# zyc-123/InstanceDiff

Hardware: AMD Instinct MI355X
Metric: denoising steps/sec (256x256 bs16) (higher is better)
Workload: dtype f32; 1 GPU; 256x256 1-ch synthetic, 1000-step reverse chain, batch 16 per GPU, 2 UNet fwd + reverse update per step; global_batch=16, parallelism=replicas x1 (no collective)

## Files before the change

### include/idiff.h

```cpp
#ifndef IDIFF_H
#define IDIFF_H

#include <stdint.h>

#ifdef __cplusplus
extern "C" {
#endif

#define IDIFF_OK 0
#define IDIFF_E_BADARG (-1)
#define IDIFF_E_UNSUPPORTED (-2)
#define IDIFF_E_HIP (-3)

typedef void* idiff_stream_t;

const char* idiff_last_error(void);
int idiff_version(void);
int64_t idiff_launch_count(void);
int idiff_device_info(int* num_cu, int* wave_size, char* arch_name, int arch_name_len);

#define IDIFF_CONV_NORMAL 0
#define IDIFF_CONV_UPSAMPLE2 1
#define IDIFF_CONV_UNSHUFFLE2 2

typedef struct {
    const float* src0;
    const float* src1;
    int64_t src0_bstride, src1_bstride;
    int32_t C0, C1;
    int32_t B, Hin, Win;
    int32_t mode;
    int32_t ks;
    int32_t Cout;
    const float* wpk;
    const float* bias;
    const float* pro_a;
    const float* pro_b;
    float* out;
    int64_t out_bstride;
    const float* res;
    int64_t res_bstride;
    const float* vec;
    const float* aux;
    int64_t aux_bstride;
    const float* aux_a;
    const float* aux_b;
    float* stats;
    const float* wwino;
    const float* wwino4;
    const float* gn_gamma;
    const float* gn_beta;
    const float* gn_film;
    int64_t gn_film_ld;
    float gn_eps;
    int32_t gn_groups;
    float* gn_out_a;
    float* gn_out_b;
    float* gn_mean_rstd;
    int32_t algo_request;
    const void* wx3;
    const void* wbf16;
    int32_t operands;
} idiff_conv_desc;

int idiff_conv2d_num_tiles(int Hout, int Wout);
int idiff_conv2d_fwd(const idiff_conv_desc* d, idiff_stream_t stream);
#define IDIFF_CONV_ALGO_DIRECT 0
#define IDIFF_CONV_ALGO_WINOGRAD 1
#define IDIFF_CONV_ALGO_STREAM1X1 2
#define IDIFF_CONV_ALGO_WINOGRAD4 3
#define IDIFF_CONV_ALGO_WINOGRAD4H 4
#define IDIFF_CONV_ALGO_X3 5
#define IDIFF_CONV_ALGO_BF16 6
int idiff_conv2d_last_algo(void);
int idiff_conv2d_plan(const idiff_conv_desc* d);
long long idiff_conv1x1_x3_image_bytes(int Cout, int Cin);
int idiff_pack_conv1x1_x3(const float* w, void* image, int Cout, int Cin, idiff_stream_t stream);
int idiff_pack_conv_weight(const float* w, float* wpk, int Cout, int Cin, int ks, idiff_stream_t stream);
int idiff_pack_conv_weight_T(const float* w, float* wpk, int Cout, int Cin, int ks, idiff_stream_t stream);
int idiff_pack_conv_weight_wino(const float* w, float* wwino, int Cout, int Cin, int transpose, idiff_stream_t stream);
int idiff_pack_conv_weight_wino4(const float* w, float* wwino4, int Cout, int Cin, int transpose, idiff_stream_t stream);
long long idiff_conv_weight_bf16_bytes(int Cout, int Cin, int transpose);
int idiff_pack_conv_weight_bf16(const float* w, void* image, int Cout, int Cin, int transpose, idiff_stream_t stream);

int idiff_gn_finalize(const float* stats, int ntiles, int B, int C, int groups, int HW, const float* gamma,
                      const float* beta, const float* film, int64_t film_ld, float eps, float* out_a, float* out_b,
                      float* mean_rstd, idiff_stream_t stream);

int idiff_affine_silu_add(const float* h, int64_t h_bstride, const float* a, const float* b, const float* res,
                          int64_t res_bstride, const float* vec, float* out, int64_t out_bstride, int B, int C, int HW,
                          idiff_stream_t stream);

#define IDIFF_ACT_NONE 0
#define IDIFF_ACT_SILU 1
#define IDIFF_ACT_GELU 2
int idiff_linear_fwd(const float* x, int64_t ldx, const float* w, int64_t ldw, const float* bias, const float* res,
                     int64_t ldr, const float* gscale, float* out, int64_t ldo, int R, int K, int N, int act_in,
                     int act_out, idiff_stream_t stream);
int idiff_linear_t_fwd(const float* x, int64_t ldx, const float* wT, int64_t ldw, const float* bias, const float* res,
                       int64_t ldr, const float* gscale, float* out, int64_t ldo, int R, int K, int N, int act_in,
                       int act_out, idiff_stream_t stream);
#define IDIFF_LINEAR_MAX_GROUPS 16
typedef struct {
    const float* x;
    int64_t ldx;
    const float* wT;
    int64_t ldw;
    const float* bias;
    const float* res;
    int64_t ldr;
    const float* gscale;
    float* out;
    int64_t ldo;
    const float* ln_g;
    const float* ln_b;
    float ln_eps;
    int32_t R, K, N, act_in, act_out;
} idiff_linear_group;
int idiff_linear_t_grouped_fwd(const idiff_linear_group* groups, int ngroups, idiff_stream_t stream);
int idiff_linear_t_ln_fwd(const float* x, int64_t ldx, const float* ln_g, const float* ln_b, float ln_eps, const float* wT,
                          int64_t ldw, const float* bias, const float* res, int64_t ldr, const float* gscale, float* out,
                          int64_t ldo, int R, int K, int N, int act_out, idiff_stream_t stream);
int idiff_linear_t_heads_fwd(const float* x, int64_t ldx, int64_t x_hs, const float* wT, int64_t ldw, int64_t w_hs,
                             const float* bias, int64_t b_hs, float* out, int64_t ldo, int64_t o_hs, int R, int K, int N,
                             int heads, idiff_stream_t stream);
int idiff_smm_memproj_fwd(const float* feat, int64_t feat_bstride, const float* ln1_g, const float* ln1_b,
                          const float* wpk, const float* bias, const float* ln2_g, const float* ln2_b, float* out, int B,
                          int C, int N, float eps, idiff_stream_t stream);
int idiff_smm_memproj_compact_fwd(const float* feat, int64_t feat_bstride, const float* ln1_g, const float* ln1_b,
                                  const float* gram, const float* hvec, float evar, float* out, int B, int C, int N, int Cm,
                                  float eps1, float eps2, idiff_stream_t stream);
int idiff_smm_memproj_compact_train_fwd(const float* feat, int64_t feat_bstride, const float* ln1_g, const float* ln1_b, const float* gram,
                                        const float* hvec, const float* evar_dev, float* out, int B, int C, int N, int Cm, float eps1,
                                        float eps2, idiff_stream_t stream);
int64_t idiff_smm_memproj_compact_bwd_ws_floats(int B, int C, int N);
int idiff_smm_memproj_compact_bwd(const float* feat, int64_t feat_bstride, const float* ln1_g, const float* ln1_b, const float* gram,
                                  const float* hvec, const float* evar_dev, const float* dm, float* dfeat, int64_t dfeat_bstride,
                                  float* dparams, float* ws, int B, int C, int N, int Cm, float eps1, float eps2, idiff_stream_t stream);
#define IDIFF_MEMPROJ_MAX_GROUPS 4
typedef struct idiff_memproj_group {
    const float* feat;
    int64_t feat_bstride;
    const float *ln1_g, *ln1_b, *gram, *hvec;
    float evar;
    float* out;
    int32_t C, N, Cm;
} idiff_memproj_group;
int idiff_smm_memproj_compact_grouped_fwd(const idiff_memproj_group* groups, int ngroups, int B, float eps1, float eps2,
                                          idiff_stream_t stream);
int idiff_layernorm_rows_fwd(const float* x, int64_t ldx, const float* gamma, const float* beta, float* out,
                             int64_t ldo, int R, int C, float eps, float* mean_rstd, idiff_stream_t stream);
int idiff_time_embed_fwd(const float* t, const float* freqs, int B, int dim, float* out, idiff_stream_t stream);
int idiff_time_mlp_fwd(const float* t, const float* freqs, const float* w0, const float* b0, const float* w2, const float* b2, float* out,
                       int B, int dim, int hid, int nout, idiff_stream_t stream);

int idiff_chan_layernorm_fwd(const float* x, int64_t x_bstride, const float* gamma, const float* beta, float* out,
                             int64_t out_bstride, int B, int C, int HW, float eps, float* mean_rstd,
                             idiff_stream_t stream);

int idiff_attn_self_fwd(const float* qkv, float* out, float* lse, int B, int C, int N, int heads, float scale,
                        idiff_stream_t stream);
int idiff_attn_self_bf16_fwd(const float* qkv, float* out, int B, int C, int N, int heads, float scale, idiff_stream_t stream);
int idiff_attn_self_f16_fwd(const float* qkv, float* out, int B, int C, int N, int heads, float scale, idiff_stream_t stream);
int idiff_attn_ctx_fwd(const float* q, const float* k, const float* v, float* out, int B, int C, int N, int M,
                       int heads, float scale, idiff_stream_t stream);
int idiff_attn_tokens_fwd(const float* q, const float* k, const float* v, float* out, int B, int Nq, int M, int C,
                          int heads, float scale, int64_t ldq, int64_t ldkv, idiff_stream_t stream);
int idiff_attn_tokens_bwd(const float* q, const float* k, const float* v, const float* d_o, float* dq, float* dk, float* dv, int B, int Nq,
                          int M, int C, int heads, float scale, int64_t ldq, int64_t ldkv, int64_t ldo, int64_t lddq, int64_t lddkv,
                          idiff_stream_t stream);
int idiff_attn_tokens_grouped_fwd(const float* const* q, const float* const* k, const float* const* v, float* const* out, int ngroups,
                                  int B, int Nq, int M, int C, int heads, float scale, int64_t ldq, int64_t ldkv, idiff_stream_t stream);
int idiff_attn_tokens_f16_fwd(const float* q, const float* k, const float* v, float* out, int B, int Nq, int M, int C, int heads, float scale,
                              int64_t ldq, int64_t ldkv, idiff_stream_t stream);
int64_t idiff_smm_xattn_kv_f16_ws_floats(int B, int N);
int idiff_smm_xattn_kv_f16_fwd(const float* q, const float* k, const float* v, float* out, float* ws, int B, int Nq, int heads, int C, int N,
                               float scale, idiff_stream_t stream);
int64_t idiff_smm_xattn_ws_floats(int B, int Nq, int heads, int Cm, int N);
int idiff_smm_xattn_fwd(const float* qf, const float* mem, float* o, float* ws, int B, int Nq, int heads, int Cm,
                        int N, float scale, idiff_stream_t stream);
#define IDIFF_XATTN_MAX_GROUPS 8
typedef struct idiff_xattn_group {
    const float* qf;
    const float* mem;
    float* o;
    float* ws;
    int32_t Cm, N;
} idiff_xattn_group;
int idiff_smm_xattn_grouped_fwd(const idiff_xattn_group* groups, int ngroups, int B, int Nq, int heads, float scale,
                                idiff_stream_t stream);
int idiff_smm_xattn_lse_fwd(const float* qf, const float* mem, float* o, float* lse, float* ws, int B, int rows, int N, float scale,
                            idiff_stream_t stream);
int idiff_smm_xattn_bwd(const float* qf, const float* mem, const float* o, const float* lse, const float* d_o, float* dqf, float* dmem,
                        int accumulate, float* ws, int B, int rows, int N, float scale, idiff_stream_t stream);
int idiff_smm_xattn_cm_lse_fwd(const float* qf, const float* mem, float* o, float* lse, float* ws, int B, int rows, int Cm, int N,
                               float scale, idiff_stream_t stream);
int idiff_smm_xattn_cm_bwd(const float* qf, const float* mem, const float* o, const float* lse, const float* d_o, float* dqf, float* dmem,
                           int accumulate, float* ws, int B, int rows, int Cm, int N, float scale, idiff_stream_t stream);
int idiff_scoremap_fwd(const float* feat, int64_t feat_bstride, const float* tv, float* out, const int32_t* idx,
                       float* sel, int B, int C, int HW, int K, idiff_stream_t stream);
#define IDIFF_SCOREMAP_MAX_GROUPS 4
typedef struct idiff_scoremap_group {
    const float* feat;
    int64_t feat_bstride;
    const float* tv;
    float* out;
    float* sel;
    int32_t C, HW;
} idiff_scoremap_group;
int idiff_scoremap_grouped_fwd(const idiff_scoremap_group* groups, int ngroups, const int32_t* idx, int B, int K, idiff_stream_t stream);
int idiff_conv3x3_select_fwd(const float* x, int64_t x_bstride, const float* w, const float* bias, const int32_t* idx, float* out,
                             int B, int C, int K, int H, int W, idiff_stream_t stream);
int64_t idiff_conv3x3_select_bwd_ws_floats(int B, int C, int H, int W);
int idiff_conv3x3_select_bwd(const float* x, int64_t x_bstride, const float* w, const int32_t* idx, const float* dpred, float* dx,
                             int64_t dx_bstride, float* dw, float* db, float* ws, int B, int C, int K, int H, int W, idiff_stream_t stream);
int idiff_gather_channel(const float* x, const int32_t* idx, float* out, int B, int C, int HW, idiff_stream_t stream);

#define IDIFF_SDE_STEP 0
#define IDIFF_SDE_MEAN 1
#define IDIFF_SDE_ODE 2
int idiff_irsde_reverse_step(const float* x, const float* mu, const float* noise_pred, const float* z, float* x_out,
                             int64_t n, float theta, float sigma, float sigma_bar, float dt, float sqrt_dt, int mode,
                             uint64_t seed, uint64_t offset, idiff_stream_t stream);
#define IDIFF_IRSDE_SCORE_FROM_NOISE 0
#define IDIFF_IRSDE_MU_BAR 1
#define IDIFF_IRSDE_DRIFT 2
#define IDIFF_IRSDE_REV_DRIFT 3
#define IDIFF_IRSDE_DISPERSION 4
#define IDIFF_IRSDE_STEP_MEAN 5
#define IDIFF_IRSDE_STEP_SDE 6
#define IDIFF_IRSDE_FORWARD_STEP 7
#define IDIFF_IRSDE_OPT_STEP 8
#define IDIFF_IRSDE_REAL_NOISE 9
#define IDIFF_IRSDE_REAL_SCORE 10
#define IDIFF_IRSDE_INIT_FROM_NOISE 11
#define IDIFF_IRSDE_RANDOM_STATES 12
#define IDIFF_IRSDE_NUM_OPS 13
int idiff_irsde_map(int op, const float* a, const float* b, const float* z, const float* mu, float mu_scalar, float* out, int B,
                    int64_t per_sample, const float* coef_dev, const float* k, uint64_t seed, uint64_t offset,
                    idiff_stream_t stream);
int idiff_drift_reverse_step(const float* x, const float* r_hat, const float* e_hat, const float* z, const float* cond,
                             float* x_out, float* xa_out, int64_t n, float a, float b, float c, uint64_t seed,
                             uint64_t offset, idiff_stream_t stream);
int idiff_drift_reverse_step_dev(float* x, const float* r_hat, const float* e_hat, const float* z_base, const float* cond,
                                 float* xa, int64_t n, const float* coef, int Tp1, const int32_t* state, uint64_t seed,
                                 uint64_t nper, uint64_t offset_base, idiff_stream_t stream);
int idiff_drift_reverse_step2_dev(float* x, const float* r_hat, const float* e_hat, float* r_prev, float* e_prev, const float* z_base,
                                  const float* cond, float* xa, int64_t n, const float* coef5, int Tp1, const int32_t* state,
                                  uint64_t seed, uint64_t nper, uint64_t offset_base, idiff_stream_t stream);
int idiff_randn_members(float* out, int R, int64_t n_s, const uint64_t* members_dev, uint64_t seed, uint64_t j, idiff_stream_t stream);
int idiff_ensemble_init(const float* cond, float* cond_rep, float* x, float* xa, int B, int S, int64_t n_s, const uint64_t* members_dev,
                        float sigma, uint64_t seed, idiff_stream_t stream);
int idiff_chain_begin(const float* cond_in, float* cond, float* x, float* xa, int B, int S, int64_t n_s, int64_t row0, int R,
                      const uint64_t* members_dev, float sigma, uint64_t seed, uint64_t offset, int32_t* state, float* tdev, int t0,
                      int calls0, idiff_stream_t stream);
int idiff_drift_reverse_step_members_dev(float* x, const float* r_hat, const float* e_hat, float* r_prev, float* e_prev, const float* z_base,
                                         const float* cond, float* xa, int R, int64_t n_s, const float* coef, int coef_rows, int Tp1,
                                         const int32_t* state, const uint64_t* members_dev, uint64_t seed, idiff_stream_t stream);
int idiff_ensemble_stats(const float* x, float* mean, float* std_out, int B, int S, int64_t n_s, idiff_stream_t stream);
int idiff_ensemble_order_stats(const float* x, float* out, int B, int S, int64_t n_s, const int32_t* ks_host, int nk, int algo,
                               idiff_stream_t stream);
int idiff_interval_coverage(const float* lo, const float* hi, const float* target, int32_t* counts, int32_t* ws, int B, int64_t n_s,
                            idiff_stream_t stream);
int64_t idiff_interval_coverage_ws_ints(int B, int64_t n_s);
int idiff_ensemble_scores(const float* x, const float* target, float* crps_map, double* sums, int32_t* counts, void* ws, int B, int S,
                          int64_t n_s, idiff_stream_t stream);
int64_t idiff_ensemble_scores_ws_bytes(int B, int S);
int idiff_tile_gather(const float* full, float* tiles, int B, int C, int H, int W, int ny, int nx, int Ph, int Pw, const int32_t* ytab,
                      const int32_t* xtab, idiff_stream_t stream);
int idiff_drift_reverse_step_tiled_dev(float* x, const float* r_tiles, const float* e_tiles, float* r_prev, float* e_prev, const float* z_base,
                                       const float* cond, float* x_tiles, float* xa_tiles, int B, int C, int H, int W, int ny, int nx, int Ph,
                                       int Pw, const int32_t* ytab, const float* ywt, const int32_t* xtab, const float* xwt, const float* coef,
                                       int coef_rows, int Tp1, const int32_t* state, uint64_t seed, uint64_t nper, uint64_t offset_base,
                                       idiff_stream_t stream);
int idiff_drift_reverse_step_tiled_members_dev(float* x, const float* r_tiles, const float* e_tiles, float* r_prev, float* e_prev,
                                               const float* z_base, const float* cond, float* x_tiles, float* xa_tiles, int R, int C, int H,
                                               int W, int ny, int nx, int Ph, int Pw, const int32_t* ytab, const float* ywt,
                                               const int32_t* xtab, const float* xwt, const float* coef, int coef_rows, int Tp1,
                                               const int32_t* state, const uint64_t* members_dev, uint64_t seed, idiff_stream_t stream);
int idiff_step_state_advance(int32_t* state, float* tdev, int B, int T, int t_stop, idiff_stream_t stream);
int idiff_step_state_advance_table(int32_t* state, float* tdev, int B, const int32_t* next_t, int Tp1, int t_first, int t_stop,
                                   idiff_stream_t stream);
int idiff_dropout(const float* x, float* out, int64_t n, float p, uint64_t seed, uint64_t offset, idiff_stream_t stream);
int idiff_randn(float* out, int64_t n, uint64_t seed, uint64_t offset, idiff_stream_t stream);
int idiff_philox_raw(uint32_t* out, int64_t ncounters, uint64_t seed, uint64_t offset, idiff_stream_t stream);
int idiff_axpby(const float* x, const float* y, float* out, int64_t n, float alpha, float beta, idiff_stream_t stream);
int idiff_sum_n(const float* const* srcs, const int64_t* src_bstrides, int nsrc, float* out, int64_t out_bstride, int B,
                int64_t per_sample, idiff_stream_t stream);
int idiff_gather_segments(const void* segs_dev, int nseg, int64_t nblocks, float* dst, idiff_stream_t stream);
int idiff_gather_segments_acc(const void* segs_dev, int nseg, int64_t nblocks, float* dst, idiff_stream_t stream);
int idiff_mix3_per_sample(const float* x0, const float* cond, const float* eps, const float* c0, const float* c1,
                          const float* c2, float* out, int B, int64_t per_sample, idiff_stream_t stream);


int64_t idiff_conv2d_wgrad_ws_floats(const idiff_conv_desc* d);
int idiff_conv2d_wgrad(const idiff_conv_desc* d, const float* dy, int64_t dy_bstride, float* dw, int accumulate, float* ws,
                       idiff_stream_t stream);
int idiff_conv2d_wgrad_last_algo(void);
int idiff_sumpool2x2(const float* x, float* out, int64_t planes, int h, int w, idiff_stream_t stream);
int idiff_pixel_shuffle2(const float* x, float* out, int B, int C, int h, int w, idiff_stream_t stream);
int idiff_plane_sum(const float* x, int64_t x_bstride, float* out_bc, int B, int C, int HW, idiff_stream_t stream);
int idiff_batch_sum(const float* in_bc, float* out_c, int B, int C, int accumulate, idiff_stream_t stream);

int64_t idiff_gn_silu_bwd_ws_floats(int B, int C, int groups);
int idiff_gn_silu_bwd(const float* dy, int64_t dy_bstride, const float* h, int64_t h_bstride, const float* a, const float* b,
                      const float* mean_rstd, const float* gamma, const float* beta, const float* film, int64_t film_ld,
                      float* dh, int64_t dh_bstride, float* dgamma, float* dbeta, float* dfilm, int64_t dfilm_ld, float* ws,
                      int B, int C, int groups, int HW, int accumulate, float* dh_sum, float* dy_sum, idiff_stream_t stream);

int idiff_act_fwd(const float* x, float* y, int64_t n, int act, idiff_stream_t stream);
int idiff_act_bwd(const float* dy, const float* x, float* dx, int64_t n, int act, idiff_stream_t stream);
int idiff_colsum(const float* x, int64_t ldx, float* out, int R, int N, int accumulate, idiff_stream_t stream);
int idiff_scale_cols(const float* x, const float* g, float* out, int R, int N, idiff_stream_t stream);
int idiff_colsum_prod(const float* x, const float* y, float* out, int R, int N, idiff_stream_t stream);
int idiff_layernorm_rows_g_fwd(const float* x, int64_t ldx, const float* gamma, const float* beta, float* out, int64_t ldo, int R, int C,
                               float eps, float* mean_rstd, int groups, idiff_stream_t stream);
int idiff_layernorm_rows_g_bwd(const float* dy, int64_t lddy, const float* x, int64_t ldx, const float* gamma, const float* mean_rstd,
                               float* dx, int64_t lddx, float* dgamma, float* dbeta, int R, int C, int groups, idiff_stream_t stream);
int idiff_colsum_g(const float* x, int64_t ldx, float* out, int R, int N, int groups, idiff_stream_t stream);
int idiff_layernorm_rows_bwd(const float* dy, int64_t lddy, const float* x, int64_t ldx, const float* gamma,
                             const float* mean_rstd, float* dx, int64_t lddx, float* dgamma, float* dbeta, int R, int C,
                             int accumulate, idiff_stream_t stream);
int64_t idiff_chan_layernorm_bwd_ws_floats(int B, int C, int HW);
int idiff_chan_layernorm_bwd(const float* dy, int64_t dy_bstride, const float* x, int64_t x_bstride, const float* gamma,
                             const float* mean_rstd, float* dx, int64_t dx_bstride, float* dgamma, float* dbeta, float* ws,
                             int B, int C, int HW, int accumulate, idiff_stream_t stream);
int idiff_chan_normalize_fwd(const float* x, int64_t x_bstride, float* y, float* nrm, int B, int C, int HW,
                             idiff_stream_t stream);
int idiff_chan_normalize_bwd(const float* dy, const float* y, const float* nrm, float* dx, int64_t dx_bstride, int B, int C,
                             int HW, idiff_stream_t stream);
int idiff_scatter_channel(const float* x, const int32_t* idx, float* out, int B, int C, int HW, idiff_stream_t stream);

int64_t idiff_bgemm_ws_floats(int M, int N, int K, int batch);
int idiff_bgemm(const float* A, const float* B, float* C, int M, int N, int K, int64_t lda, int64_t ldb, int64_t ldc,
                int transA, int transB, int64_t sA, int64_t sB, int64_t sC, int batch, float alpha, float beta, float* ws,
                idiff_stream_t stream);
int idiff_bgemm_bias(const float* A, const float* B, float* C, int M, int N, int K, int64_t lda, int64_t ldb, int64_t ldc, int transA,
                     int transB, int64_t sA, int64_t sB, int64_t sC, int batch, float alpha, const float* colbias, int64_t sbias,
                     idiff_stream_t stream);
int idiff_linear_mfma_fwd(const float* x, int64_t ldx, const float* w, int64_t ldw, const float* bias, float* out, int64_t ldo, int R,
                          int K, int N, idiff_stream_t stream);
int idiff_softmax_rows_fwd(const float* x, int64_t ldx, float* out, int64_t ldo, int R, int N, float scale,
                           idiff_stream_t stream);
int idiff_softmax_rows_bwd(const float* p, int64_t ldp, const float* dp, int64_t lddp, float* ds, int64_t ldds, int R, int N,
                           float scale, idiff_stream_t stream);

int idiff_resize_bilinear(const float* x, float* out, int64_t planes, int H, int W, int oh, int ow, idiff_stream_t stream);
int idiff_mse_loss(const float* a, const float* b, float* loss, float* grad, float* ws, int64_t n, float grad_scale,
                   idiff_stream_t stream);
int idiff_image_metrics(const float* pred, const float* target, float* out_b3, float* ws, int B, int H, int W,
                        idiff_stream_t stream);
int idiff_adam_step(float* p, const float* g, float* m, float* v, int64_t n, float lr, float beta1, float beta2, float eps,
                    float weight_decay, float grad_scale, int step, idiff_stream_t stream);

int64_t idiff_grad_sumsq_parts(void);
int idiff_grad_sumsq(const float* g, int64_t n, float* part , idiff_stream_t stream);
int idiff_grad_guard(const float* part, int nbuf, float grad_scale, float max_norm, int skip_nonfinite, float* info ,
                     idiff_stream_t stream);
int idiff_adam_step_dev(float* p, const float* g, float* m, float* v, int64_t n, float lr, float beta1, float beta2, float eps,
                        float weight_decay, float grad_scale, int step, const float* info, idiff_stream_t stream);

int idiff_f32_to_bf16(const float* x, uint16_t* out, int64_t n, idiff_stream_t stream);
int idiff_bf16_to_f32(const uint16_t* x, float* out, int64_t n, idiff_stream_t stream);

#ifdef __cplusplus
}
#endif
#endif
```

### instancediff_amd/_lib.py

```python
import ctypes as C
import os
import re

_HERE = os.path.dirname(os.path.abspath(__file__))
LIB_PATH = os.environ.get("IDIFF_LIB") or os.path.join(_HERE, "libidiff_hip.so")
HEADER_PATH = os.path.join(os.path.dirname(_HERE), "include", "idiff.h")

c_f32p = C.c_void_p
c_stream = C.c_void_p


class ConvDesc(C.Structure):
    _fields_ = [
        ("src0", C.c_void_p), ("src1", C.c_void_p),
        ("src0_bstride", C.c_int64), ("src1_bstride", C.c_int64),
        ("C0", C.c_int32), ("C1", C.c_int32),
        ("B", C.c_int32), ("Hin", C.c_int32), ("Win", C.c_int32),
        ("mode", C.c_int32), ("ks", C.c_int32), ("Cout", C.c_int32),
        ("wpk", C.c_void_p), ("bias", C.c_void_p),
        ("pro_a", C.c_void_p), ("pro_b", C.c_void_p),
        ("out", C.c_void_p), ("out_bstride", C.c_int64),
        ("res", C.c_void_p), ("res_bstride", C.c_int64),
        ("vec", C.c_void_p),
        ("aux", C.c_void_p), ("aux_bstride", C.c_int64), ("aux_a", C.c_void_p), ("aux_b", C.c_void_p),
        ("stats", C.c_void_p),
        ("wwino", C.c_void_p),
        ("wwino4", C.c_void_p),
        ("gn_gamma", C.c_void_p), ("gn_beta", C.c_void_p), ("gn_film", C.c_void_p), ("gn_film_ld", C.c_int64), ("gn_eps", C.c_float),
        ("gn_groups", C.c_int32), ("gn_out_a", C.c_void_p), ("gn_out_b", C.c_void_p), ("gn_mean_rstd", C.c_void_p),
        ("algo_request", C.c_int32),
        ("wx3", C.c_void_p),
        ("wbf16", C.c_void_p), ("operands", C.c_int32),
    ]


class LinearGroup(C.Structure):
    _fields_ = [("x", C.c_void_p), ("ldx", C.c_int64), ("wT", C.c_void_p), ("ldw", C.c_int64), ("bias", C.c_void_p), ("res", C.c_void_p),
                ("ldr", C.c_int64), ("gscale", C.c_void_p), ("out", C.c_void_p), ("ldo", C.c_int64), ("ln_g", C.c_void_p), ("ln_b", C.c_void_p),
                ("ln_eps", C.c_float), ("R", C.c_int32), ("K", C.c_int32), ("N", C.c_int32), ("act_in", C.c_int32), ("act_out", C.c_int32)]


class XattnGroup(C.Structure):
    _fields_ = [("qf", C.c_void_p), ("mem", C.c_void_p), ("o", C.c_void_p), ("ws", C.c_void_p), ("Cm", C.c_int32), ("N", C.c_int32)]


class MemprojGroup(C.Structure):
    _fields_ = [("feat", C.c_void_p), ("feat_bstride", C.c_int64), ("ln1_g", C.c_void_p), ("ln1_b", C.c_void_p), ("gram", C.c_void_p),
                ("hvec", C.c_void_p), ("evar", C.c_float), ("out", C.c_void_p), ("C", C.c_int32), ("N", C.c_int32), ("Cm", C.c_int32)]


class ScoremapGroup(C.Structure):
    _fields_ = [("feat", C.c_void_p), ("feat_bstride", C.c_int64), ("tv", C.c_void_p), ("out", C.c_void_p), ("sel", C.c_void_p),
                ("C", C.c_int32), ("HW", C.c_int32)]


LINEAR_MAX_GROUPS = 16
XATTN_MAX_GROUPS, MEMPROJ_MAX_GROUPS, SCOREMAP_MAX_GROUPS = 8, 4, 4
P, I, I64, F, U64 = C.c_void_p, C.c_int, C.c_int64, C.c_float, C.c_uint64

SIGNATURES = {
    "idiff_last_error": (C.c_char_p, []),
    "idiff_version": (I, []),
    "idiff_launch_count": (I64, []),
    "idiff_device_info": (I, [C.POINTER(I), C.POINTER(I), C.c_char_p, I]),
    "idiff_conv2d_num_tiles": (I, [I, I]),
    "idiff_conv2d_fwd": (I, [C.POINTER(ConvDesc), c_stream]),
    "idiff_conv2d_last_algo": (I, []),
    "idiff_conv2d_plan": (I, [C.POINTER(ConvDesc)]),
    "idiff_pack_conv_weight": (I, [P, P, I, I, I, c_stream]),
    "idiff_pack_conv_weight_T": (I, [P, P, I, I, I, c_stream]),
    "idiff_pack_conv_weight_wino": (I, [P, P, I, I, I, c_stream]),
    "idiff_pack_conv_weight_wino4": (I, [P, P, I, I, I, c_stream]),
    "idiff_conv_weight_bf16_bytes": (C.c_longlong, [I, I, I]),
    "idiff_pack_conv_weight_bf16": (I, [P, P, I, I, I, c_stream]),
    "idiff_conv1x1_x3_image_bytes": (C.c_longlong, [I, I]),
    "idiff_pack_conv1x1_x3": (I, [P, P, I, I, c_stream]),
    "idiff_gn_finalize": (I, [P, I, I, I, I, I, P, P, P, I64, F, P, P, P, c_stream]),
    "idiff_affine_silu_add": (I, [P, I64, P, P, P, I64, P, P, I64, I, I, I, c_stream]),
    "idiff_linear_fwd": (I, [P, I64, P, I64, P, P, I64, P, P, I64, I, I, I, I, I, c_stream]),
    "idiff_linear_t_fwd": (I, [P, I64, P, I64, P, P, I64, P, P, I64, I, I, I, I, I, c_stream]),
    "idiff_linear_t_ln_fwd": (I, [P, I64, P, P, F, P, I64, P, P, I64, P, P, I64, I, I, I, I, c_stream]),
    "idiff_linear_t_grouped_fwd": (I, [C.POINTER(LinearGroup), I, c_stream]),
    "idiff_attn_tokens_grouped_fwd": (I, [C.POINTER(P), C.POINTER(P), C.POINTER(P), C.POINTER(P), I, I, I, I, I, I, F, I64, I64, c_stream]),
    "idiff_linear_t_heads_fwd": (I, [P, I64, I64, P, I64, I64, P, I64, P, I64, I64, I, I, I, I, c_stream]),
    "idiff_smm_memproj_fwd": (I, [P, I64, P, P, P, P, P, P, P, I, I, I, F, c_stream]),
    "idiff_smm_memproj_compact_fwd": (I, [P, I64, P, P, P, P, F, P, I, I, I, I, F, F, c_stream]),
    "idiff_smm_memproj_compact_train_fwd": (I, [P, I64, P, P, P, P, P, P, I, I, I, I, F, F, c_stream]),
    "idiff_smm_memproj_compact_bwd_ws_floats": (I64, [I, I, I]),
    "idiff_smm_memproj_compact_bwd": (I, [P, I64, P, P, P, P, P, P, P, I64, P, P, I, I, I, I, F, F, c_stream]),
    "idiff_smm_memproj_compact_grouped_fwd": (I, [C.POINTER(MemprojGroup), I, I, F, F, c_stream]),
    "idiff_layernorm_rows_fwd": (I, [P, I64, P, P, P, I64, I, I, F, P, c_stream]),
    "idiff_time_embed_fwd": (I, [P, P, I, I, P, c_stream]),
    "idiff_time_mlp_fwd": (I, [P, P, P, P, P, P, P, I, I, I, I, c_stream]),
    "idiff_chan_layernorm_fwd": (I, [P, I64, P, P, P, I64, I, I, I, F, P, c_stream]),
    "idiff_attn_self_fwd": (I, [P, P, P, I, I, I, I, F, c_stream]),
    "idiff_attn_self_bf16_fwd": (I, [P, P, I, I, I, I, F, c_stream]),
    "idiff_attn_self_f16_fwd": (I, [P, P, I, I, I, I, F, c_stream]),
    "idiff_attn_ctx_fwd": (I, [P, P, P, P, I, I, I, I, I, F, c_stream]),
    "idiff_attn_tokens_fwd": (I, [P, P, P, P, I, I, I, I, I, F, I64, I64, c_stream]),
    "idiff_attn_tokens_bwd": (I, [P, P, P, P, P, P, P, I, I, I, I, I, F, I64, I64, I64, I64, I64, c_stream]),
    "idiff_smm_xattn_ws_floats": (I64, [I, I, I, I, I]),
    "idiff_attn_tokens_f16_fwd": (I, [P, P, P, P, I, I, I, I, I, F, I64, I64, c_stream]),
    "idiff_smm_xattn_kv_f16_ws_floats": (I64, [I, I]),
    "idiff_smm_xattn_kv_f16_fwd": (I, [P, P, P, P, P, I, I, I, I, I, F, c_stream]),
    "idiff_smm_xattn_fwd": (I, [P, P, P, P, I, I, I, I, I, F, c_stream]),
    "idiff_smm_xattn_grouped_fwd": (I, [C.POINTER(XattnGroup), I, I, I, I, F, c_stream]),
    "idiff_smm_xattn_lse_fwd": (I, [P, P, P, P, P, I, I, I, F, c_stream]),
    "idiff_smm_xattn_bwd": (I, [P, P, P, P, P, P, P, I, P, I, I, I, F, c_stream]),
    "idiff_smm_xattn_cm_lse_fwd": (I, [P, P, P, P, P, I, I, I, I, F, c_stream]),
    "idiff_smm_xattn_cm_bwd": (I, [P, P, P, P, P, P, P, I, P, I, I, I, I, F, c_stream]),
    "idiff_scoremap_fwd": (I, [P, I64, P, P, P, P, I, I, I, I, c_stream]),
    "idiff_scoremap_grouped_fwd": (I, [C.POINTER(ScoremapGroup), I, P, I, I, c_stream]),
    "idiff_gather_channel": (I, [P, P, P, I, I, I, c_stream]),
    "idiff_conv3x3_select_fwd": (I, [P, I64, P, P, P, P, I, I, I, I, I, c_stream]),
    "idiff_conv3x3_select_bwd_ws_floats": (I64, [I, I, I, I]),
    "idiff_conv3x3_select_bwd": (I, [P, I64, P, P, P, P, I64, P, P, P, I, I, I, I, I, c_stream]),
    "idiff_irsde_reverse_step": (I, [P, P, P, P, P, I64, F, F, F, F, F, I, U64, U64, c_stream]),
    "idiff_irsde_map": (I, [I, P, P, P, P, F, P, I, I64, P, C.POINTER(C.c_float), U64, U64, c_stream]),
    "idiff_drift_reverse_step": (I, [P, P, P, P, P, P, P, I64, F, F, F, U64, U64, c_stream]),
    "idiff_drift_reverse_step_dev": (I, [P, P, P, P, P, P, I64, P, I, P, U64, U64, U64, c_stream]),
    "idiff_drift_reverse_step2_dev": (I, [P, P, P, P, P, P, P, P, I64, P, I, P, U64, U64, U64, c_stream]),
    "idiff_randn_members": (I, [P, I, I64, P, U64, U64, c_stream]),
    "idiff_ensemble_init": (I, [P, P, P, P, I, I, I64, P, F, U64, c_stream]),
    "idiff_chain_begin": (I, [P, P, P, P, I, I, I64, I64, I, P, F, U64, U64, P, P, I, I, c_stream]),
    "idiff_drift_reverse_step_members_dev": (I, [P, P, P, P, P, P, P, P, I, I64, P, I, I, P, P, U64, c_stream]),
    "idiff_ensemble_stats": (I, [P, P, P, I, I, I64, c_stream]),
    "idiff_ensemble_order_stats": (I, [P, P, I, I, I64, C.POINTER(C.c_int32), I, I, c_stream]),
    "idiff_interval_coverage": (I, [P, P, P, P, P, I, I64, c_stream]),
    "idiff_interval_coverage_ws_ints": (I64, [I, I64]),
    "idiff_ensemble_scores": (I, [P, P, P, P, P, P, I, I, I64, c_stream]),
    "idiff_ensemble_scores_ws_bytes": (I64, [I, I]),
    "idiff_tile_gather": (I, [P, P, I, I, I, I, I, I, I, I, P, P, c_stream]),
    "idiff_drift_reverse_step_tiled_dev": (I, [P, P, P, P, P, P, P, P, P, I, I, I, I, I, I, I, I, P, P, P, P, P, I, I, P, U64, U64, U64, c_stream]),
    "idiff_drift_reverse_step_tiled_members_dev": (I, [P, P, P, P, P, P, P, P, P, I, I, I, I, I, I, I, I, P, P, P, P, P, I, I, P, P, U64, c_stream]),
    "idiff_step_state_advance": (I, [P, P, I, I, I, c_stream]),
    "idiff_step_state_advance_table": (I, [P, P, I, P, I, I, I, c_stream]),
    "idiff_randn": (I, [P, I64, U64, U64, c_stream]),
    "idiff_dropout": (I, [P, P, I64, F, U64, U64, c_stream]),
    "idiff_philox_raw": (I, [P, I64, U64, U64, c_stream]),
    "idiff_axpby": (I, [P, P, P, I64, F, F, c_stream]),
    "idiff_mix3_per_sample": (I, [P, P, P, P, P, P, P, I, I64, c_stream]),
    "idiff_conv2d_wgrad_ws_floats": (I64, [C.POINTER(ConvDesc)]),
    "idiff_conv2d_wgrad": (I, [C.POINTER(ConvDesc), P, I64, P, I, P, c_stream]),
    "idiff_conv2d_wgrad_last_algo": (I, []),
    "idiff_sumpool2x2": (I, [P, P, I64, I, I, c_stream]),
    "idiff_pixel_shuffle2": (I, [P, P, I, I, I, I, c_stream]),
    "idiff_plane_sum": (I, [P, I64, P, I, I, I, c_stream]),
    "idiff_batch_sum": (I, [P, P, I, I, I, c_stream]),
    "idiff_sum_n": (I, [C.POINTER(P), C.POINTER(I64), I, P, I64, I, I64, c_stream]),
    "idiff_gather_segments": (I, [P, I, I64, P, c_stream]),
    "idiff_gather_segments_acc": (I, [P, I, I64, P, c_stream]),
    "idiff_gn_silu_bwd_ws_floats": (I64, [I, I, I]),
    "idiff_gn_silu_bwd": (I, [P, I64, P, I64, P, P, P, P, P, P, I64, P, I64, P, P, P, I64, P, I, I, I, I, I, P, P, c_stream]),
    "idiff_act_fwd": (I, [P, P, I64, I, c_stream]),
    "idiff_act_bwd": (I, [P, P, P, I64, I, c_stream]),
    "idiff_colsum": (I, [P, I64, P, I, I, I, c_stream]),
    "idiff_scale_cols": (I, [P, P, P, I, I, c_stream]),
    "idiff_colsum_prod": (I, [P, P, P, I, I, c_stream]),
    "idiff_layernorm_rows_bwd": (I, [P, I64, P, I64, P, P, P, I64, P, P, I, I, I, c_stream]),
    "idiff_chan_layernorm_bwd_ws_floats": (I64, [I, I, I]),
    "idiff_chan_layernorm_bwd": (I, [P, I64, P, I64, P, P, P, I64, P, P, P, I, I, I, I, c_stream]),
    "idiff_chan_normalize_fwd": (I, [P, I64, P, P, I, I, I, c_stream]),
    "idiff_chan_normalize_bwd": (I, [P, P, P, P, I64, I, I, I, c_stream]),
    "idiff_scatter_channel": (I, [P, P, P, I, I, I, c_stream]),
    "idiff_bgemm_ws_floats": (I64, [I, I, I, I]),
    "idiff_bgemm": (I, [P, P, P, I, I, I, I64, I64, I64, I, I, I64, I64, I64, I, F, F, P, c_stream]),
    "idiff_bgemm_bias": (I, [P, P, P, I, I, I, I64, I64, I64, I, I, I64, I64, I64, I, F, P, I64, c_stream]),
    "idiff_layernorm_rows_g_fwd": (I, [P, I64, P, P, P, I64, I, I, F, P, I, c_stream]),
    "idiff_layernorm_rows_g_bwd": (I, [P, I64, P, I64, P, P, P, I64, P, P, I, I, I, c_stream]),
    "idiff_colsum_g": (I, [P, I64, P, I, I, I, c_stream]),
    "idiff_linear_mfma_fwd": (I, [P, I64, P, I64, P, P, I64, I, I, I, c_stream]),
    "idiff_softmax_rows_fwd": (I, [P, I64, P, I64, I, I, F, c_stream]),
    "idiff_softmax_rows_bwd": (I, [P, I64, P, I64, P, I64, I, I, F, c_stream]),
    "idiff_resize_bilinear": (I, [P, P, I64, I, I, I, I, c_stream]),
    "idiff_mse_loss": (I, [P, P, P, P, P, I64, F, c_stream]),
    "idiff_image_metrics": (I, [P, P, P, P, I, I, I, c_stream]),
    "idiff_f32_to_bf16": (I, [P, P, I64, c_stream]),
    "idiff_bf16_to_f32": (I, [P, P, I64, c_stream]),
    "idiff_adam_step": (I, [P, P, P, P, I64, F, F, F, F, F, F, I, c_stream]),
    "idiff_grad_sumsq_parts": (I64, []),
    "idiff_grad_sumsq": (I, [P, I64, P, c_stream]),
    "idiff_grad_guard": (I, [P, I, F, F, I, P, c_stream]),
    "idiff_adam_step_dev": (I, [P, P, P, P, I64, F, F, F, F, F, F, I, P, c_stream]),
}


def header_symbols(path=HEADER_PATH):
    with open(path) as f:
        txt = f.read()
    txt = re.sub(r"/\*.*?\*/", "", txt, flags=re.S)
    return sorted(set(re.findall(r"\b(idiff_[A-Za-z0-9_]+)\s*\(", txt)))


class IdiffError(RuntimeError):
    pass


_lib = None


def load():
    global _lib
    if _lib is not None:
        return _lib
    if not os.path.exists(LIB_PATH):
        raise IdiffError(
            f"{LIB_PATH} not found: the HIP kernel library has not been built. Run `python -c 'import __graft_entry__ as g; "
            "g.build()'` (or `make -C instancediff_amd/csrc`). There is no CPU fallback.")
    lib = C.CDLL(LIB_PATH)
    for name, (res, args) in SIGNATURES.items():
        try:
            fn = getattr(lib, name)
        except AttributeError as e:
            raise IdiffError(f"libidiff_hip.so does not export {name}; rebuild it") from e
        fn.restype = res
        fn.argtypes = args
    _lib = lib
    return lib


def check(rc, what=""):
    if rc != 0:
        msg = load().idiff_last_error()
        raise IdiffError(f"{what} failed ({rc}): {msg.decode() if msg else ''}")
```

### instancediff_amd/csrc/conv_args.h

```cpp
#pragma once
#include "common.h"

namespace idiff_detail {

struct ConvShape {
    int C0v, C1v, Cin, Hout, Wout;
};
inline const char* conv_shape(const idiff_conv_desc* d, ConvShape* s) {
    const bool unsh = d->mode == IDIFF_CONV_UNSHUFFLE2, ups = d->mode == IDIFF_CONV_UPSAMPLE2;
    s->C0v = unsh ? d->C0 * 4 : d->C0;
    s->C1v = d->C1;
    s->Cin = s->C0v + s->C1v;
    s->Hout = ups ? d->Hin * 2 : (unsh ? d->Hin / 2 : d->Hin);
    s->Wout = ups ? d->Win * 2 : (unsh ? d->Win / 2 : d->Win);
    if (unsh && !(d->ks == 1 && d->C1 == 0)) return "unshuffle mode needs ks=1 and a single source";
    if (unsh && !(d->Hin % 2 == 0 && d->Win % 2 == 0)) return "unshuffle needs even H, W";
    return nullptr;
}

struct GnTail {
    const float* gamma;
    const float* beta;
    const float* film;
    long long film_ld;
    float eps;
    int groups;
    float* out_a;
    float* out_b;
    float* mean_rstd;
};

struct ConvArgs {
    const float* src0;
    const float* src1;
    long long bs0, bs1;
    int C0v, C1v;
    int C0r;
    int Cin;
    int B, Hin, Win, Hout, Wout;
    int Cout;
    const float* wpk;
    const float* wwino;
    const float* wwino4;
    const float* bias;
    const float* pro_a;
    const float* pro_b;
    float* out;
    long long obs;
    const float* res;
    long long rbs;
    const float* vec;
    const float* aux;
    long long abs_;
    const float* aux_a;
    const float* aux_b;
    float* stats;
    GnTail gn;
    int tiles_x, ntiles, ncob;
    unsigned total_wg;
};

bool conv_wino_eligible(const ConvArgs& a, int ks, int mode);
int launch_conv_wino(const ConvArgs& a, int mode, hipStream_t st);

long long conv_wino4_items(const ConvArgs& a, int ks, int mode, bool requested = false);
int launch_conv_wino4(const ConvArgs& a, int mode, hipStream_t st);
int launch_conv_wino4h(const ConvArgs& a, int mode, hipStream_t st);

bool conv1x1_x3_eligible(const ConvArgs& a, int mode);
int launch_conv1x1_x3(const ConvArgs& a, int mode, const void* wx3, hipStream_t st);

bool conv_bf16_eligible(const ConvArgs& a, int ks, int mode, const void* wbf16);
int launch_conv_bf16(const ConvArgs& a, int mode, const void* wbf16, hipStream_t st);

}
```

### instancediff_amd/csrc/conv_igemm.hip

```cpp
#include <stdlib.h>

#include <type_traits>

#include "conv_args.h"

using idiff_detail::ConvArgs;

namespace {

typedef float floatx2 __attribute__((ext_vector_type(2)));

template <int KS, int CK, int TWL, int MODE, bool VECW, int MB, int SPEC>
__global__ __launch_bounds__(256) void conv_igemm_kernel(const ConvArgs a) {
    constexpr int BM = 32 * MB;
    constexpr int TW = 1 << TWL;
    constexpr int TH = 256 / TW;
    constexpr int PAD = KS / 2;
    constexpr int TRH = TH + KS - 1;
    constexpr int RS = TW + KS - 1;
    constexpr int PS = TRH * RS;
    constexpr int IN_TILE = ((CK * PS + 3) / 4) * 4;
    constexpr int TAPS = KS * KS;
    constexpr int W_TILE = TAPS * CK * BM;
    constexpr int BUF = IN_TILE + W_TILE;
// ... 293 lines not shown
            auto fetch = [&](int i) {
                const int f = tid + i * 256;
                const int row = mb * 32 + (f >> 6), c4 = (f & 63) * 4;
                const long long o = (co0 + row < a.Cout) ? (long long)(co0 + row) * HWo + pix0 + c4 : pix0 + c4;
                if (RES) nres = *reinterpret_cast<const floatx4*>(resb + o);
                if (AUX) naux = *reinterpret_cast<const floatx4*>(auxb + o);
            };
            fetch(0);
            __syncthreads();
#pragma unroll
            for (int r = 0; r < 16; ++r) {
                const int col = (r & 3) + 8 * (r >> 2) + 4 * half;
#pragma unroll
                for (int nb = 0; nb < 2; ++nb) ot[col * OLD + wave * 64 + nb * 32 + l31] = mb ? acc[MB - 1][nb][r] : acc[0][nb][r];
            }
            __syncthreads();
#pragma unroll
            for (int i = 0; i < STEPS; ++i) {
                const int f = tid + i * 256;
                const int lrow = f >> 6, row = mb * 32 + lrow, c4 = (f & 63) * 4;
                const floatx4 cres = nres, caux = naux;
                if (i + 1 < STEPS) fetch(i + 1);
                floatx4 v = *reinterpret_cast<const floatx4*>(ot + lrow * OLD + c4);
                const float add = econst[row] + econst[BM + row];
                v = floatx4{v.x + add, v.y + add, v.z + add, v.w + add};
                if (RES) v = floatx4{v.x + cres.x, v.y + cres.y, v.z + cres.z, v.w + cres.w};
                if (AUX) {
                    const float aa = econst[2 * BM + row], ab = econst[3 * BM + row];
                    v = floatx4{v.x + silu_fast(aa * caux.x + ab), v.y + silu_fast(aa * caux.y + ab), v.z + silu_fast(aa * caux.z + ab),
                                v.w + silu_fast(aa * caux.w + ab)};
                }
                if (co0 + row < a.Cout) *reinterpret_cast<floatx4*>(outb + (long long)(co0 + row) * HWo + pix0 + c4) = v;
            }
        };
        auto halves = [&](auto res_tag, auto aux_tag) {
#pragma unroll
            for (int mb = 0; mb < MB; ++mb) rows(mb, res_tag, aux_tag);
        };
        if (has_res) {
            if (has_aux) halves(std::true_type{}, std::true_type{});
            else halves(std::true_type{}, std::false_type{});
        } else {
            if (has_aux) halves(std::false_type{}, std::true_type{});
            else halves(std::false_type{}, std::false_type{});
        }
        return;
    }

    float sv[MB * 32];
    auto out_steps = [&](auto res_tag, auto aux_tag) {
        constexpr bool RES = decltype(res_tag)::value, AUX = decltype(aux_tag)::value;
        float nres[2], naux[2];
        auto fetch = [&](int i) {
            const int co = co0 + (i >> 4) * 32 + (i & 3) + 8 * ((i & 15) >> 2) + 4 * half;
#pragma unroll
            for (int nb = 0; nb < 2; ++nb) {
                const long long o = (pval[nb] && co < a.Cout) ? (long long)co * HWo + opix[nb] : 0;
                if (RES) nres[nb] = resb[o];
                if (AUX) naux[nb] = auxb[o];
            }
        };
        fetch(0);
#pragma unroll
        for (int i = 0; i < MB * 16; ++i) {
            const int mb = i >> 4, r = i & 15;
            const int col = mb * 32 + (r & 3) + 8 * (r >> 2) + 4 * half;
            const int co = co0 + col;
            const bool cval = co < a.Cout;
            const float cres[2] = {nres[0], nres[1]}, caux[2] = {naux[0], naux[1]};
            if (i + 1 < MB * 16) fetch(i + 1);
            const float bv = econst[col], add = econst[BM + col];
            float aa = 0.f, ab = 0.f;
            if (AUX) aa = econst[2 * BM + col], ab = econst[3 * BM + col];
            float s = 0.f, q = 0.f;
#pragma unroll
            for (int nb = 0; nb < 2; ++nb) {
                float v = acc[mb][nb][r] + bv;
                if (pval[nb] && cval) {
                    s += v;
                    q += v * v;
                    v += add;
                    if (RES) v += cres[nb];
                    if (AUX) v += silu_fast(aa * caux[nb] + ab);
                    outb[(long long)co * HWo + opix[nb]] = v;
                }
            }
            sv[i * 2 + 0] = s;
            sv[i * 2 + 1] = q;
        }
    };
    if (resb) {
        if (auxb) out_steps(std::true_type{}, std::true_type{});
        else out_steps(std::true_type{}, std::false_type{});
    } else {
        if (auxb) out_steps(std::false_type{}, std::true_type{});
        else out_steps(std::false_type{}, std::false_type{});
    }
    if (want_stats) {
        constexpr int NV = MB * 32;
#pragma unroll
        for (int step = 0; step < 5; ++step) {
            const int m = 16 >> step;
            const int n = NV >> (step + 1);
            if (n >= 1) {
                const bool up = (l31 & m) != 0;
#pragma unroll
                for (int j = 0; j < n; ++j) {
                    const float lo = sv[j], hi = sv[j + n];
                    const float send = up ? lo : hi;
                    const float keep = up ? hi : lo;
                    sv[j] = keep + __shfl_xor(send, m, 64);
                }
            }
        }
        if (MB == 2) {
            const int mbq = l31 >> 4, r = l31 & 15;
            const int col = mbq * 32 + (r & 3) + 8 * (r >> 2) + 4 * half;
            red[(wave * BM + col) * 2 + 0] = sv[0];
            red[(wave * BM + col) * 2 + 1] = sv[1];
        } else {
            const int r = l31 >> 1, w = l31 & 1;
            const int col = (r & 3) + 8 * (r >> 2) + 4 * half;
            red[(wave * BM + col) * 2 + w] = sv[0];
        }
        __syncthreads();
        if (tid < BM * 2) {
            const int col = tid >> 1, w = tid & 1;
            const int co = co0 + col;
            if (co < a.Cout) {
                const float t = red[(0 * BM + col) * 2 + w] + red[(1 * BM + col) * 2 + w] + red[(2 * BM + col) * 2 + w] +
                                red[(3 * BM + col) * 2 + w];
                a.stats[(((long long)b * a.ntiles + tile) * a.Cout + co) * 2 + w] = t;
            }
        }
    }
}

template <int KS, int CK, int TWL, int MODE, bool VECW, int MB, int SPEC>
int launch_conv(const ConvArgs& a, hipStream_t st) {
    constexpr int BM = 32 * MB;
    constexpr int TW = 1 << TWL;
    constexpr int TH = 256 / TW;
    constexpr int TRH = TH + KS - 1;
    constexpr int RS = TW + KS - 1;
    constexpr int IN_TILE = ((CK * TRH * RS + 3) / 4) * 4;
    constexpr int W_TILE = KS * KS * CK * BM;
    size_t taboff = (size_t)2 * (IN_TILE + W_TILE);
    if (KS == 1 && TWL == 8 && MODE == IDIFF_CONV_NORMAL && (size_t)32 * 260 > taboff) taboff = (size_t)32 * 260;
    const size_t lds = (taboff + (a.pro_a ? 2 * (size_t)a.C0r : 0) + 4 * BM) * sizeof(float);
    static idiff_dyn_lds_cache lds_cache;
    auto kern = conv_igemm_kernel<KS, CK, TWL, MODE, VECW, MB, SPEC>;
    if (const int rc = idiff_dyn_lds(lds_cache, kern, lds, "conv2d")) return rc;
    hipLaunchKernelGGL(kern, dim3(a.total_wg), dim3(256), lds, st, a);
    IDIFF_CHECK_LAUNCH("conv2d_fwd");
    return IDIFF_OK;
}

template <int KS, int CK, int MODE, int MB>
int dispatch_tw(const ConvArgs& a, int twl, bool vecw, hipStream_t st) {
    if (twl == 8) {
        if constexpr (KS == 1 && MODE == IDIFF_CONV_NORMAL && MB == 2) {
            if (!vecw) IDIFF_FAIL(IDIFF_E_UNSUPPORTED, "conv2d: internal: flattened tile needs vector weights");
            if (a.pro_a) return launch_conv<1, CK, 8, IDIFF_CONV_NORMAL, true, 2, 2>(a, st);
            if (a.src1) return launch_conv<1, CK, 8, IDIFF_CONV_NORMAL, true, 2, 3>(a, st);
            return launch_conv<1, CK, 8, IDIFF_CONV_NORMAL, true, 2, 1>(a, st);
        }
        IDIFF_FAIL(IDIFF_E_UNSUPPORTED, "conv2d: internal: flattened tile requested for an unsupported variant");
    }
    if (twl == 5) {
        if (KS == 3 && MODE == IDIFF_CONV_NORMAL && MB == 2 && vecw) {
            if (a.pro_a) return launch_conv<KS, CK, 5, MODE, true, MB, 2>(a, st);
            if (a.src1) return launch_conv<KS, CK, 5, MODE, true, MB, 3>(a, st);
            return launch_conv<KS, CK, 5, MODE, true, MB, 1>(a, st);
        }
        return vecw ? launch_conv<KS, CK, 5, MODE, true, MB, 0>(a, st) : launch_conv<KS, CK, 5, MODE, false, MB, 0>(a, st);
    }
    if (twl == 4) return vecw ? launch_conv<KS, CK, 4, MODE, true, MB, 0>(a, st) : launch_conv<KS, CK, 4, MODE, false, MB, 0>(a, st);
    return vecw ? launch_conv<KS, CK, 3, MODE, true, MB, 0>(a, st) : launch_conv<KS, CK, 3, MODE, false, MB, 0>(a, st);
}

template <int KS, int CK, int MODE>
int dispatch_mb(const ConvArgs& a, int twl, int mb, bool vecw, hipStream_t st) {
    return mb == 2 ? dispatch_tw<KS, CK, MODE, 2>(a, twl, vecw, st) : dispatch_tw<KS, CK, MODE, 1>(a, twl, vecw, st);
}

inline int pick_twl(int Wout) { return Wout >= 24 ? 5 : (Wout >= 16 ? 4 : 3); }

__global__ void pack_weight_kernel(const float* __restrict__ w, float* __restrict__ out, int Cout, int Cin, int taps, int transpose) {
    const long long n = (long long)Cout * Cin * taps;
    for (long long i = blockIdx.x * (long long)blockDim.x + threadIdx.x; i < n; i += (long long)gridDim.x * blockDim.x) {
        if (!transpose) {
            const int co = i % Cout;
            const int ci = (i / Cout) % Cin;
            const int tap = i / ((long long)Cout * Cin);
            out[i] = w[((long long)co * Cin + ci) * taps + tap];
        } else {
            const int ci = i % Cin;
            const int co = (i / Cin) % Cout;
            const int tap = i / ((long long)Cout * Cin);
            out[i] = w[((long long)co * Cin + ci) * taps + (taps - 1 - tap)];
        }
    }
}

}

static thread_local int g_last_algo = IDIFF_CONV_ALGO_DIRECT;
extern "C" int idiff_conv2d_last_algo(void) { return g_last_algo; }

extern "C" int idiff_conv2d_num_tiles(int Hout, int Wout) {
    const int twl = pick_twl(Wout);
    const int TW = 1 << twl, TH = 256 / TW;
    return ((Wout + TW - 1) / TW) * ((Hout + TH - 1) / TH);
}

struct ConvPlan {
    int algo;
    ConvArgs a;
    int twl, mb;
    bool vecw;
};

static int conv2d_args(const idiff_conv_desc* d, ConvPlan* p) {
    IDIFF_CHECK_ARG(d && d->src0 && d->wpk && d->out, "conv2d: null pointer");
    IDIFF_CHECK_ARG(d->B > 0 && d->C0 > 0 && d->Cout > 0 && d->Hin > 0 && d->Win > 0, "conv2d: bad dims");
    IDIFF_CHECK_ARG(d->ks == 1 || d->ks == 3 || d->ks == 7, "conv2d: ks must be 1, 3 or 7 (got %d)", d->ks);
    IDIFF_CHECK_ARG(d->mode >= 0 && d->mode <= 2, "conv2d: bad mode %d", d->mode);
    IDIFF_CHECK_ARG((d->C1 > 0) == (d->src1 != nullptr), "conv2d: src1/C1 mismatch");
    IDIFF_CHECK_ARG(!(d->pro_a && d->C1 > 0), "conv2d: prologue needs a single source");
    IDIFF_CHECK_ARG((d->pro_a == nullptr) == (d->pro_b == nullptr), "conv2d: pro_a/pro_b must both be set");
    IDIFF_CHECK_ARG(!d->aux || (d->aux_a && d->aux_b), "conv2d: aux needs aux_a/aux_b");
    ConvArgs& a = p->a;
    a.src0 = d->src0;
    a.src1 = d->src1;
    a.bs0 = d->src0_bstride;
    a.bs1 = d->src1_bstride;
    a.B = d->B;
    a.C0r = d->C0;
    a.Hin = d->Hin;
    a.Win = d->Win;
    a.Cout = d->Cout;
    a.wpk = d->wpk;
    a.wwino = d->wwino;
    a.wwino4 = d->wwino4;
    a.bias = d->bias;
    a.pro_a = d->pro_a;
    a.pro_b = d->pro_b;
    a.out = d->out;
    a.obs = d->out_bstride;
    a.res = d->res;
    a.rbs = d->res_bstride;
    a.vec = d->vec;
    a.aux = d->aux;
    a.abs_ = d->aux_bstride;
    a.aux_a = d->aux_a;
    a.aux_b = d->aux_b;
    a.stats = d->stats;
    memset(&a.gn, 0, sizeof(a.gn));
    if (d->gn_out_a) {
        IDIFF_CHECK_ARG(d->stats && d->gn_out_b && d->gn_groups > 0 && d->Cout % d->gn_groups == 0 && d->Cout / d->gn_groups <= 256,
                        "conv2d: GroupNorm finalize needs stats, gn_out_b and groups dividing Cout (<= 256 channels per group)");
        a.gn.gamma = d->gn_gamma, a.gn.beta = d->gn_beta, a.gn.film = d->gn_film, a.gn.film_ld = d->gn_film_ld, a.gn.eps = d->gn_eps;
        a.gn.groups = d->gn_groups, a.gn.out_a = d->gn_out_a, a.gn.out_b = d->gn_out_b, a.gn.mean_rstd = d->gn_mean_rstd;
    }
    idiff_detail::ConvShape s;
    if (const char* why = idiff_detail::conv_shape(d, &s)) IDIFF_FAIL(IDIFF_E_BADARG, "conv2d: %s", why);
    a.C0v = s.C0v, a.C1v = s.C1v, a.Cin = s.Cin, a.Hout = s.Hout, a.Wout = s.Wout;
    IDIFF_CHECK_ARG(a.bs0 >= (long long)d->C0 * d->Hin * d->Win, "conv2d: src0_bstride too small");
    IDIFF_CHECK_ARG(d->C1 == 0 || a.bs1 >= (long long)d->C1 * d->Hin * d->Win, "conv2d: src1_bstride too small");
    IDIFF_CHECK_ARG(a.obs >= (long long)d->Cout * a.Hout * a.Wout, "conv2d: out_bstride too small");
    int twl = pick_twl(a.Wout);
    const int mb = p->mb = a.Cout <= 32 ? 1 : 2;
    const bool vecw = p->vecw = (a.Cout % 4 == 0) && ((reinterpret_cast<uintptr_t>(a.wpk) & 15) == 0);
    const bool in16 = (reinterpret_cast<uintptr_t>(a.src0) & 15) == 0 && (reinterpret_cast<uintptr_t>(a.src1) & 15) == 0 && a.bs0 % 4 == 0 &&
                      (!a.src1 || a.bs1 % 4 == 0);
    if (d->ks == 1 && d->mode == IDIFF_CONV_NORMAL && !a.stats && mb == 2 && vecw && in16 && ((long long)a.Hout * a.Wout) % 256 == 0 &&
        a.Wout >= 32) {
        a.Win = a.Wout = a.Hout * a.Wout;
        a.Hin = a.Hout = 1;
        twl = 8;
    }
    const int TW = 1 << twl, TH = 256 / TW;
    const int bm = 32 * mb;
    a.tiles_x = (a.Wout + TW - 1) / TW;
    a.ntiles = a.tiles_x * ((a.Hout + TH - 1) / TH);
    a.ncob = (a.Cout + bm - 1) / bm;
    const long long total = (long long)a.B * a.ntiles * a.ncob;
    IDIFF_CHECK_ARG(total < (1ll << 31), "conv2d: grid too large");
    a.total_wg = (unsigned)total;
    p->twl = twl;
    return IDIFF_OK;
}

static int conv2d_choose(const idiff_conv_desc* d, ConvPlan* p) {
    const ConvArgs& a = p->a;
    const int twl = p->twl;
    auto take = [p](int algo) {
        p->algo = algo;
        return IDIFF_OK;
    };
    const bool hard = d->algo_request > 0;
    const int req = (hard ? d->algo_request : -d->algo_request) - 1;
    IDIFF_CHECK_ARG(req == -1 || req == IDIFF_CONV_ALGO_DIRECT || req == IDIFF_CONV_ALGO_WINOGRAD || req == IDIFF_CONV_ALGO_WINOGRAD4 ||
                        req == IDIFF_CONV_ALGO_WINOGRAD4H || req == IDIFF_CONV_ALGO_X3 || req == IDIFF_CONV_ALGO_BF16,
                    "conv2d: bad algo_request %d", d->algo_request);
    IDIFF_CHECK_ARG(d->operands == 0 || d->operands == 1, "conv2d: bad operands %d", d->operands);
    {
        const bool reqbf = req == IDIFF_CONV_ALGO_BF16;
        const bool can = idiff_detail::conv_bf16_eligible(a, d->ks, d->mode, d->wbf16);
        IDIFF_CHECK_ARG(!(hard && reqbf) || can, "conv2d: algo_request bf16 but the layer is not a 3x3 that tiles for it (Cout %% 64, C0 / C1 %% 32, "
                        "Hout %% 8, Wout %% 32) or has no bf16 image");
        if (can && (reqbf || (req == -1 && d->operands == 1))) return take(IDIFF_CONV_ALGO_BF16);
    }
    {
        static const bool x3_on = [] {
            const char* e = getenv("IDIFF_X3");
            return !e || atoi(e) != 0;
        }();
        const bool reqx3 = req == IDIFF_CONV_ALGO_X3;
        bool can = false;
        ConvArgs ax = a;
        if (d->ks == 1 && d->wx3 != nullptr && (reinterpret_cast<uintptr_t>(d->wx3) & 15) == 0) {
            if (d->mode == IDIFF_CONV_NORMAL) {
                can = twl == 8 && idiff_detail::conv1x1_x3_eligible(ax, d->mode);
            } else if (d->mode == IDIFF_CONV_UNSHUFFLE2) {
                ax.ncob = a.Cout / 64;
                ax.ntiles = (int)(((long long)a.Hout * a.Wout) / 256);
                ax.tiles_x = ax.ntiles;
                const long long tot = (long long)a.B * ax.ntiles * ax.ncob;
                ax.total_wg = (unsigned)tot;
                can = tot > 0 && tot < (1ll << 31) && idiff_detail::conv1x1_x3_eligible(ax, d->mode);
            }
        }
        IDIFF_CHECK_ARG(!(hard && reqx3) || can, "conv2d: algo_request bf16x3 but the layer is not a 1x1 that tiles by 256 pixels with a split weight image");
        if (can && (reqx3 || (req == -1 && x3_on))) {
            p->a = ax;
            return take(IDIFF_CONV_ALGO_X3);
        }
    }
    static const int w4h_mode = [] {
        const char* e = getenv("IDIFF_W4H");
        return e ? atoi(e) : 1;
    }();
    const bool req4 = req == IDIFF_CONV_ALGO_WINOGRAD4, req4h = req == IDIFF_CONV_ALGO_WINOGRAD4H;
    const long long items16 = (req == -1 || req4 || req4h) ? idiff_detail::conv_wino4_items(a, d->ks, d->mode, req4 || req4h) : 0;
    if (items16 > 0) {
        const long long items8 = (long long)a.ntiles * a.ncob;
        const bool w4_ok = a.Cin >= 16;
        IDIFF_CHECK_ARG(!(hard && req4) || w4_ok, "conv2d: algo_request F(4x4,3x3) 16x32-item kernel needs Cin >= 16 (got %d)", a.Cin);
        bool half;
        if (req4h) half = true;
        else if (req4 && w4_ok) half = false;
        else if (items16 >= 16 && w4_ok) half = w4h_mode == 2 || (w4h_mode == 3 && a.src1 != nullptr);
        else half = w4h_mode >= 1 && items8 >= 16;
        if (half) return take(IDIFF_CONV_ALGO_WINOGRAD4H);
        if (w4_ok && (req4 || items16 >= 16)) return take(IDIFF_CONV_ALGO_WINOGRAD4);
    }
    IDIFF_CHECK_ARG(!hard || !(req4 || req4h), "conv2d: algo_request F(4x4,3x3) but the shape does not tile for it");
    if ((req == -1 || req == IDIFF_CONV_ALGO_WINOGRAD || !hard) && req != IDIFF_CONV_ALGO_DIRECT && idiff_detail::conv_wino_eligible(a, d->ks, d->mode))
        return take(IDIFF_CONV_ALGO_WINOGRAD);
    IDIFF_CHECK_ARG(!hard || req != IDIFF_CONV_ALGO_WINOGRAD, "conv2d: algo_request F(2x2,3x3) but the shape does not tile for it");
    IDIFF_CHECK_ARG(!(d->ks == 1 && d->mode == IDIFF_CONV_UPSAMPLE2), "conv2d: upsample mode needs ks=3");
    IDIFF_CHECK_ARG(d->ks != 7 || d->mode == IDIFF_CONV_NORMAL, "conv2d: ks=7 needs normal mode");
    return take(IDIFF_CONV_ALGO_DIRECT);
}

static int conv2d_launch(const idiff_conv_desc* d, const ConvPlan& p, idiff_stream_t stream) {
    const ConvArgs& a = p.a;
    hipStream_t st = (hipStream_t)stream;
    const bool normal = d->mode == IDIFF_CONV_NORMAL;
    int rc;
    switch (p.algo) {
        case IDIFF_CONV_ALGO_X3: return idiff_detail::launch_conv1x1_x3(a, d->mode, d->wx3, st);
        case IDIFF_CONV_ALGO_BF16: rc = idiff_detail::launch_conv_bf16(a, d->mode, d->wbf16, st); break;
        case IDIFF_CONV_ALGO_WINOGRAD4H: rc = idiff_detail::launch_conv_wino4h(a, d->mode, st); break;
        case IDIFF_CONV_ALGO_WINOGRAD4: rc = idiff_detail::launch_conv_wino4(a, d->mode, st); break;
        case IDIFF_CONV_ALGO_WINOGRAD: rc = idiff_detail::launch_conv_wino(a, d->mode, st); break;
        default:
            if (d->ks == 3)
                rc = normal ? dispatch_mb<3, 8, IDIFF_CONV_NORMAL>(a, p.twl, p.mb, p.vecw, st) : dispatch_mb<3, 8, IDIFF_CONV_UPSAMPLE2>(a, p.twl, p.mb, p.vecw, st);
            else if (d->ks == 1)
                rc = normal ? dispatch_mb<1, 16, IDIFF_CONV_NORMAL>(a, p.twl, p.mb, p.vecw, st) : dispatch_mb<1, 16, IDIFF_CONV_UNSHUFFLE2>(a, p.twl, p.mb, p.vecw, st);
            else
                rc = dispatch_mb<7, 2, IDIFF_CONV_NORMAL>(a, p.twl, p.mb, p.vecw, st);
    }
    if (rc != IDIFF_OK || !d->gn_out_a) return rc;
    return idiff_gn_finalize(d->stats, a.ntiles, a.B, a.Cout, d->gn_groups, a.Hout * a.Wout, d->gn_gamma, d->gn_beta, d->gn_film, d->gn_film_ld,
                             d->gn_eps, d->gn_out_a, d->gn_out_b, d->gn_mean_rstd, stream);
}

extern "C" int idiff_conv2d_fwd(const idiff_conv_desc* d, idiff_stream_t stream) {
    ConvPlan p;
    if (const int rc = conv2d_args(d, &p)) return rc;
    if (const int rc = conv2d_choose(d, &p)) return rc;
    g_last_algo = p.algo;
    return conv2d_launch(d, p, stream);
}

extern "C" int idiff_conv2d_plan(const idiff_conv_desc* d) {
    ConvPlan p;
    if (const int rc = conv2d_args(d, &p)) return rc;
    if (const int rc = conv2d_choose(d, &p)) return rc;
    return p.algo;
}

static int pack_common(const float* w, float* wpk, int Cout, int Cin, int ks, int tr, idiff_stream_t stream) {
    IDIFF_CHECK_ARG(w && wpk && Cout > 0 && Cin > 0 && ks > 0, "pack_conv_weight: bad args");
    const long long n = (long long)Cout * Cin * ks * ks;
    const int grid = (int)((n + 255) / 256 > 4096 ? 4096 : (n + 255) / 256);
    hipLaunchKernelGGL(pack_weight_kernel, dim3(grid), dim3(256), 0, (hipStream_t)stream, w, wpk, Cout, Cin, ks * ks, tr);
    IDIFF_CHECK_LAUNCH("pack_conv_weight");
    return IDIFF_OK;
}
extern "C" int idiff_pack_conv_weight(const float* w, float* wpk, int Cout, int Cin, int ks, idiff_stream_t stream) {
    return pack_common(w, wpk, Cout, Cin, ks, 0, stream);
}
extern "C" int idiff_pack_conv_weight_T(const float* w, float* wpk, int Cout, int Cin, int ks, idiff_stream_t stream) {
    return pack_common(w, wpk, Cout, Cin, ks, 1, stream);
}
```

### instancediff_amd/csrc/wino_common.h

```cpp
#pragma once
#include <stdlib.h>

#include <type_traits>

#include "common.h"

namespace idiff_detail {
bool winograd_disabled();
}

namespace idiff_wino {


template <int CTRL>
__device__ __forceinline__ float dpp_row_shr(float v) {
    return __builtin_bit_cast(float, __builtin_amdgcn_update_dpp(0, __builtin_bit_cast(int, v), CTRL, 0xf, 0xf, true));
}
__device__ __forceinline__ float row_sum16(float v) {
    v += dpp_row_shr<0x111>(v);
    v += dpp_row_shr<0x112>(v);
    v += dpp_row_shr<0x114>(v);
    v += dpp_row_shr<0x118>(v);
    return v;
}

template <typename T>
__device__ __forceinline__ T* scalar_ptr(const T* p) {
    const unsigned long long v = reinterpret_cast<unsigned long long>(p);
    const unsigned lo = __builtin_amdgcn_readfirstlane((unsigned)v), hi = __builtin_amdgcn_readfirstlane((unsigned)(v >> 32));
    return reinterpret_cast<T*>(((unsigned long long)hi << 32) | lo);
}


__host__ __device__ constexpr int PF(int u) { return (3 * u + 1) / 2; }
__host__ __device__ constexpr int PH(int u) { return 1 + 3 * (u / 2); }
__host__ __device__ constexpr int pos(int u, int v) { return v < 4 ? 4 * PF(u) + v : 4 * PH(u) + 2 * (u & 1) + (v - 4); }

__device__ __forceinline__ void bt6(const float (&x)[6], float (&o)[6]) {
    o[0] = __builtin_fmaf(4.f, x[0], __builtin_fmaf(-5.f, x[2], x[4]));
    const float p = __builtin_fmaf(-4.f, x[2], x[4]), q = __builtin_fmaf(-4.f, x[1], x[3]);
    o[1] = p + q;
    o[2] = p - q;
    const float c = x[4] - x[2], e = x[3] - x[1];
    o[3] = __builtin_fmaf(2.f, e, c);
    o[4] = __builtin_fmaf(-2.f, e, c);
    o[5] = __builtin_fmaf(4.f, x[1], __builtin_fmaf(-5.f, x[3], x[5]));
}
__device__ __forceinline__ void at6(const float x0, const float x1, const float x2, const float x3, const float x4, const float x5, float (&o)[4]) {
    const float s1 = x1 + x2, d1 = x1 - x2, s2 = x3 + x4, d2 = x3 - x4;
    o[0] = (x0 + s1) + s2;
    o[1] = __builtin_fmaf(2.f, d2, d1);
    o[2] = __builtin_fmaf(4.f, s2, s1);
    o[3] = __builtin_fmaf(8.f, d2, d1) + x5;
}
__device__ __forceinline__ void a6(float x0, float x1, float x2, float x3, float (&o)[6]) {
    const float s = x0 + x2, t = x1 + x3;
    o[0] = x0;
    o[1] = s + t;
    o[2] = s - t;
    const float p = __builtin_fmaf(4.f, x2, x0), q = __builtin_fmaf(8.f, x3, 2.f * x1);
    o[3] = p + q;
    o[4] = p - q;
    o[5] = x3;
}
__device__ __forceinline__ void g6(float x0, float x1, float x2, float (&o)[6]) {
    o[0] = 0.25f * x0;
    const float s = x0 + x2;
    o[1] = (-1.f / 6.f) * (s + x1);
    o[2] = (-1.f / 6.f) * (s - x1);
    const float t = __builtin_fmaf(4.f, x2, x0);
    o[3] = (1.f / 24.f) * __builtin_fmaf(2.f, x1, t);
    o[4] = (1.f / 24.f) * __builtin_fmaf(-2.f, x1, t);
    o[5] = x2;
}
__device__ __forceinline__ void gt3(float m0, float m1, float m2, float m3, float m4, float m5, float (&o)[3]) {
    const float s12 = m1 + m2, d12 = m1 - m2, s34 = m3 + m4, d34 = m3 - m4;
    o[0] = __builtin_fmaf(0.25f, m0, __builtin_fmaf(-1.f / 6.f, s12, (1.f / 24.f) * s34));
    o[1] = __builtin_fmaf(-1.f / 6.f, d12, (1.f / 12.f) * d34);
    o[2] = __builtin_fmaf(-1.f / 6.f, s12, __builtin_fmaf(1.f / 6.f, s34, m5));
}

template <int MODE, int NT, int NL, int PSP, int PS, int RS, int RCOLS, typename Args>
__device__ __forceinline__ void gather_decode(const int& tid, unsigned& om, const int& y0, const int& x0, const Args& a, int* const& gtab, const int& HWin) {
    int t = tid;
    asm volatile("" : "+v"(t));
    om = 0;
#pragma unroll
    for (int i = 0; i < NL; ++i) {
        const int e = t + i * NT;
        const int ci = e / PSP;
        const int rem = e - ci * PSP;
        const int r = rem / RS;
        const int c = rem - r * RS;
        const int oy = y0 - 1 + r, ox = x0 - 1 + c;
        const bool in = rem < PS && c < RCOLS && (unsigned)oy < (unsigned)a.Hout && (unsigned)ox < (unsigned)a.Wout;
        const int sp = MODE == IDIFF_CONV_UPSAMPLE2 ? (oy >> 1) * a.Win + (ox >> 1) : oy * a.Win + ox;
        gtab[i * NT + tid] = in ? (ci * HWin + sp) * 4 : -1;
        om |= (in ? 0u : 1u) << i;
    }
}

__device__ __forceinline__ void load_taps(const float* __restrict__ w, int Cin, int co, int ci, int transpose, float (&g)[3][3]) {
#pragma unroll
    for (int p = 0; p < 3; ++p)
#pragma unroll
        for (int q = 0; q < 3; ++q)
            g[p][q] = transpose ? w[((long long)ci * Cin + co) * 9 + (2 - p) * 3 + (2 - q)] : w[((long long)co * Cin + ci) * 9 + p * 3 + q];
}


template <int NPOS, typename K>
int pack_entry(const char* name, K kern, const float* w, float* image, int Cout, int Cin, int transpose, idiff_stream_t stream) {
    IDIFF_CHECK_ARG(w && image && Cout > 0 && Cin > 0, "%s: bad args", name);
    const int Co = transpose ? Cin : Cout, Ci = transpose ? Cout : Cin;
    IDIFF_CHECK_ARG(Co % 16 == 0 && Ci % 8 == 0, "%s: needs conv Cout %% 16 == 0 and Cin %% 8 == 0 (got %d, %d)", name, Co, Ci);
    if (Co % 64) {
        hipError_t e = hipMemsetAsync(image, 0, (size_t)NPOS * Ci * ((Co + 63) / 64) * 64 * sizeof(float), (hipStream_t)stream);
        if (e != hipSuccess) IDIFF_FAIL(IDIFF_E_HIP, "%s: hipMemsetAsync: %s", name, hipGetErrorString(e));
    }
    const long long n = (long long)Cout * Cin;
    const int grid = (int)((n + 255) / 256 > 4096 ? 4096 : (n + 255) / 256);
    hipLaunchKernelGGL(kern, dim3(grid), dim3(256), 0, (hipStream_t)stream, w, image, Cout, Cin, transpose);
    IDIFF_CHECK_LAUNCH(name);
    return IDIFF_OK;
}

inline int persistent_grid(int total, int slots, int* per_out = nullptr) {
    const int per = (total + slots - 1) / slots;
    if (per_out) *per_out = per;
    return (total + per - 1) / per;
}

template <typename F>
int launch_spec_ladder(int mode, bool pro, bool src1, bool ragged, F&& launch) {
    auto rag = [&](auto mode_tag, auto spec_tag) {
        if (ragged) return launch(mode_tag, spec_tag, std::true_type{});
        return launch(mode_tag, spec_tag, std::false_type{});
    };
    using Normal = std::integral_constant<int, IDIFF_CONV_NORMAL>;
    using Upsample = std::integral_constant<int, IDIFF_CONV_UPSAMPLE2>;
    if (mode == IDIFF_CONV_UPSAMPLE2) return rag(Upsample{}, std::integral_constant<int, 1>{});
    if (pro) return rag(Normal{}, std::integral_constant<int, 2>{});
    if (src1) return rag(Normal{}, std::integral_constant<int, 3>{});
    return rag(Normal{}, std::integral_constant<int, 1>{});
}

}

#ifdef IDIFF_WINO_TRACE
#define TRACE_PARAM , long long* trace
#define TRACE_INIT(N) long long tr_t[(N) + 1] = {0}, tr_acc[N] = {0};
#define TRACE_MARK(k)                       \
    tr_t[k] = __builtin_readcyclecounter(); \
    if (k > 0) tr_acc[k - 1] += tr_t[k] - tr_t[k - 1];
#define TRACE_LAP(last) \
    if (tr_t[last] != 0) tr_acc[last] += tr_t[0] - tr_t[last];
#define TRACE_FINI(N)                                                                                                   \
    if (tid == 0) {                                                                                                     \
        for (int q_ = 0; q_ < (N); ++q_) atomicAdd((unsigned long long*)trace + q_, (unsigned long long)tr_acc[q_]);    \
    }
#else
#define TRACE_PARAM
#define TRACE_INIT(N)
#define TRACE_MARK(k)
#define TRACE_LAP(last)
#define TRACE_FINI(N)
#endif
```

### instancediff_amd/models/modules/MSM_degEmb_Unet.py

```python
import math
import os
import weakref

import torch
import torch.nn as nn

from ... import ops

ARTIFACT_TYPES = ['speckle in OCT', 'speckle in ultra sound', 'noise in cryo-EM image', 'noise in low dose CT',
                  'Gaussian noise in MRI']


def _trunc_normal_(t, std=0.02):
    return nn.init.trunc_normal_(t, std=std, a=-2 * std, b=2 * std)


def _weight_epoch():
    from ... import train_ops
    return train_ops.WEIGHT_EPOCH[0]


class _Prepared:

    def __init__(self):
        self.store = weakref.WeakKeyDictionary()

    def get(self, key, params, build):
        owner, name = key[1], key[0]
        sig = (_weight_epoch(),) + tuple((p.data_ptr(), p._version) for p in params)
        slot = self.store.setdefault(owner, {})
        hit = slot.get(name)
        if hit is not None and hit[0] == sig:
            return hit[1]
        with torch.no_grad():
            val = build()
        slot[name] = (sig, val)
        return val

    def peek(self, key, params):
        owner, name = key[1], key[0]
        sig = (_weight_epoch(),) + tuple((p.data_ptr(), p._version) for p in params)
        hit = self.store.get(owner, {}).get(name)
        return hit[1] if hit is not None and hit[0] == sig else None

    def clear(self):
        self.store = weakref.WeakKeyDictionary()


_PREP = _Prepared()

SMM_SIDE = bool(int(os.environ.get("IDIFF_SMM_SIDE", "0")))
GROUPED_SMM = bool(int(os.environ.get("IDIFF_GROUPED_SMM", "1")))

def packed(conv):
    if ops.current_conv_operands() == "bf16" and tuple(conv.weight.shape[2:]) == (3, 3):
        return _PREP.get(("pk_bf16", conv), (conv.weight,), lambda: ops.pack_conv_weight(conv.weight.detach().contiguous(), bf16=True))
    return _PREP.get(("pk", conv), (conv.weight,), lambda: ops.pack_conv_weight(conv.weight.detach().contiguous()))


def wT(lin):
    return _PREP.get(("wT", lin), (lin.weight,), lambda: lin.weight.detach().t().contiguous())


class Attention(nn.Module):
    def __init__(self, dim, num_heads=8):
        super().__init__()
        self.num_heads = num_heads
        self.scale = (dim // num_heads) ** -0.5
        self.q_proj = nn.Linear(dim, dim, bias=False)
        self.k_proj = nn.Linear(dim, dim, bias=False)
        self.v_proj = nn.Linear(dim, dim, bias=False)
        self.proj = nn.Linear(dim, dim)


class TransformerDecoderLayer(nn.Module):
    def __init__(self, d_model, nhead):
        super().__init__()
        self.self_attn = Attention(d_model, nhead)
        self.cross_attn = Attention(d_model, nhead)
        self.norm1 = nn.LayerNorm(d_model)
        self.norm2 = nn.LayerNorm(d_model)
        self.norm3 = nn.LayerNorm(d_model)
        self.mlp = nn.Sequential(nn.Linear(d_model, d_model * 4), nn.GELU(), nn.Identity(), nn.Linear(d_model * 4, d_model))


class TransformerDecoderLayer_scaled(TransformerDecoderLayer):

    def __init__(self, d_model, nhead):
        super().__init__(d_model, nhead)
        self.gamma_sa = nn.Parameter(torch.ones((1, 1, d_model)) * 1e-1)
        self.gamma_ca = nn.Parameter(torch.ones((1, 1, d_model)) * 1e-1)
        self.gamma_mlp = nn.Parameter(torch.ones((1, 1, d_model)) * 1e-1)


def branch_gains(layer):
    if hasattr(layer, "gamma_sa"):
        return layer.gamma_sa.reshape(-1), layer.gamma_ca.reshape(-1), layer.gamma_mlp.reshape(-1)
    return None, None, None


class ContextDecoder(nn.Module):
    layer_cls = TransformerDecoderLayer
    if_flash = False

    def __init__(self, transformer_width=256, transformer_heads=4, transformer_layers=3, visual_dim=512, text_dim=512, dropout=0.1, outdim=None):
        super().__init__()
        self.width, self.heads = transformer_width, transformer_heads
        self.dropout = float(dropout)
        self.memory_proj = nn.Sequential(nn.LayerNorm(visual_dim), nn.Linear(visual_dim, transformer_width),
                                         nn.LayerNorm(transformer_width))
        self.text_proj = nn.Sequential(nn.LayerNorm(text_dim), nn.Linear(text_dim, transformer_width))
        self.decoder = nn.ModuleList([self.layer_cls(transformer_width, transformer_heads)
                                      for _ in range(transformer_layers)])
        self.out_proj = nn.Sequential(nn.LayerNorm(transformer_width), nn.Linear(transformer_width, visual_dim if outdim is None else outdim))
        self.apply(self._init_weights)

    @staticmethod
    def _init_weights(m):
        if isinstance(m, nn.Linear):
            _trunc_normal_(m.weight, std=.02)
            if m.bias is not None:
                nn.init.constant_(m.bias, 0)
        elif isinstance(m, nn.LayerNorm):
            nn.init.constant_(m.bias, 0)
            nn.init.constant_(m.weight, 1.0)


class ContextDecoder_Hierachical(ContextDecoder):
    layer_cls = TransformerDecoderLayer_scaled

    def __init__(self, transformer_width=256, transformer_heads=4, transformer_layers=6, visual_dim=512, text_dim=512, dropout=0.1, outdim=512,
                 if_flash=False):
        super().__init__(transformer_width, transformer_heads, transformer_layers, visual_dim, text_dim, dropout, outdim=outdim)
        self.if_flash = bool(if_flash)


DECODER_TYPES = {"ContextDecoder": ContextDecoder, "ContextDecoder_Hierachical": ContextDecoder_Hierachical}


def _class_tokens(n_cls, prompt_len, names=ARTIFACT_TYPES):
    tok = torch.zeros(n_cls, prompt_len, dtype=torch.long)
    for i in range(n_cls):
        words = (names[i] if i < len(names) else f"class {i}").split()
        tok[i, 0] = 49406
        for j, w in enumerate(words[:prompt_len - 2]):
            hsh = 0
            for ch in w:
                hsh = (hsh * 131 + ord(ch)) % 40000
            tok[i, 1 + j] = 1000 + hsh
        tok[i, min(len(words), prompt_len - 2) + 1] = 49407
    return tok


class ScoreMapModule(nn.Module):

    def __init__(self, visual_dim=64, CLIP_Type="CLIP", token_embed_dim=512, text_dim=512, n_ctx=8, n_cls=5, prompt_len=10,
                 decoder_layers=3, decoder_width=256, decoder_heads=4, tokenizer=None, class_names=ARTIFACT_TYPES, dropout=0.1,
                 decoder_type="ContextDecoder", if_flash=False):
        super().__init__()
        self.visual_dim, self.n_cls, self.text_dim = visual_dim, n_cls, text_dim
        self.contexts = nn.Parameter(torch.zeros(1, n_ctx, token_embed_dim))
        _trunc_normal_(self.contexts, std=0.02)
        self._prompt_len, self._ph_check = prompt_len, None
        self.register_buffer("tokens", _class_tokens(n_cls, prompt_len) if tokenizer is None else
                             torch.as_tensor(tokenizer(list(class_names)[:n_cls])).long())
        self.text_to_visual = nn.Linear(text_dim, visual_dim)
        if decoder_type not in DECODER_TYPES:
            raise ValueError(f"decoder_type {decoder_type!r}: expected one of {sorted(DECODER_TYPES)}")
        if if_flash and decoder_type == "ContextDecoder":
            raise ValueError("if_flash needs decoder_type ContextDecoder_Hierachical: the reference's plain TransformerDecoderLayer has no half-precision form")
        self.context_decoder = DECODER_TYPES[decoder_type](decoder_width, decoder_heads, decoder_layers, visual_dim, text_dim, dropout=dropout,
                                                           **({} if decoder_type == "ContextDecoder" else {"outdim": visual_dim, "if_flash": if_flash}))
        self.gamma = nn.Parameter(torch.ones(visual_dim) * 1e-4)
        self._text_cache = None

    def set_class_tokens(self, tokens):
        tokens = torch.as_tensor(tokens).long().to(self.tokens.device)
        assert tokens.dim() == 2 and tokens.shape[0] == self.n_cls, tokens.shape
        self.tokens = tokens
        self._text_cache = None

    def _load_from_state_dict(self, state_dict, prefix, *args, **kwargs):
        tk = state_dict.get(prefix + "tokens")
        if tk is not None and tk.shape != self.tokens.shape:
            self.tokens = torch.empty_like(tk, device=self.tokens.device)
        super()._load_from_state_dict(state_dict, prefix, *args, **kwargs)

    @property
    def tokens_are_placeholders(self):
        key = (self.tokens.data_ptr(), self.tokens._version)
        if self._ph_check is None or self._ph_check[0] != key:
            ph = _class_tokens(self.n_cls, self._prompt_len)
            self._ph_check = (key, tuple(self.tokens.shape) == tuple(ph.shape) and bool(torch.equal(self.tokens.detach().cpu(), ph)))
        return self._ph_check[1]

    def text_embeddings(self, text_encoder, B):
        if self.tokens_are_placeholders and not getattr(text_encoder, "ignores_token_ids", False):
            raise RuntimeError("ScoreMapModule holds placeholder class-token ids but the text encoder reads token ids: pass "
                               "tokenizer=... / call set_class_tokens(), or load a checkpoint that carries the `tokens` buffer")
        if not torch.is_grad_enabled() or not self.contexts.requires_grad:
            key = (B, self.contexts.data_ptr(), self.contexts._version, _weight_epoch())
            c = self._text_cache
            if c is not None and c[0] == key and c[2]() is text_encoder:
                return c[1]
            with torch.no_grad():
                text = self._encode(text_encoder).expand(B, -1, -1).contiguous()
            self._text_cache = (key, text, weakref.ref(text_encoder))
            return text
        return self._encode(text_encoder).expand(B, -1, -1).contiguous()

    def _encode(self, text_encoder):
        t = text_encoder(self.tokens, self.contexts).float()
        return t.reshape(1, self.n_cls, -1) if t.dim() == 2 else t

    def forward(self, feat, text_encoder, idx=None):
        B, C, H, W = feat.shape
        text = self.text_embeddings(text_encoder, B)
        tv = self._decoder_tokens(feat, text)
        return ops.scoremap(feat, tv.reshape(B, self.n_cls, C), idx)

    def context_decode(self, feat, text):
        B, C = feat.shape[:2]
        out = self._decoder_tokens(feat, text.contiguous(), cache_prefix=False, plain_out=True)
        return out.reshape(B, text.shape[1], -1)

    def _decoder_tokens(self, feat, text, cache_prefix=True, plain_out=False):
        return decoder_tokens_grouped([self], [feat], [text], cache_prefix=cache_prefix, plain_out=plain_out)[0]


def decoder_tokens_grouped(smms, feats, texts, cache_prefix=True, plain_out=False):
    if any(m.context_decoder.if_flash for m in smms):
        assert all(m.context_decoder.if_flash for m in smms)
        return [decoder_tokens_flash(m, f, t, plain_out=plain_out) for m, f, t in zip(smms, feats, texts)]
    L = len(smms)
    dec0 = smms[0].context_decoder
    Wd, heads, nlayers = dec0.width, dec0.heads, len(dec0.decoder)
    dh = Wd // heads
    for m in smms:
        d = m.context_decoder
        assert (d.width, d.heads, len(d.decoder)) == (Wd, heads, nlayers), "grouped ScoreMapModules must share the decoder geometry"
    dev = feats[0].device
    B = feats[0].shape[0]
    K = texts[0].shape[1]
    R = B * K

    st = []
    by_c = {}
    for m, feat, text in zip(smms, feats, texts):
        Bm, C, H, W = feat.shape
        assert Bm == B and text.shape[1] == K
        dec = m.context_decoder
        mp = dec.memory_proj
        Cm = Wd if (C + 1 > 136 or C not in (64, 128)) else (72 if C + 1 <= 72 else 136)
        compact = Cm < Wd
        mem = None
        if compact:
            gram, hvec, evar = _PREP.get(("mpvar", mp[1]), (mp[1].weight, mp[1].bias), lambda mp=mp: ops.memory_variance_form(mp[1].weight, mp[1].bias))
            by_c.setdefault((C, mp[0].eps, mp[2].eps), []).append(
                (len(st), dict(feat=feat, ln1_g=mp[0].weight, ln1_b=mp[0].bias, gram=gram, hvec=hvec, evar=evar, Cm=Cm)))
        else:
            wmp = _PREP.get(("mp", mp[1]), (mp[1].weight,),
                            lambda mp=mp, C=C: ops.pack_conv_weight(mp[1].weight.detach().reshape(Wd, C, 1, 1).contiguous()))
            mem = ops.smm_memproj(feat, mp[0].weight, mp[0].bias, wmp, mp[1].bias, mp[2].weight, mp[2].bias, eps=mp[0].eps)
        st.append(dict(m=m, dec=dec, C=C, Cm=Cm, compact=compact, mem=mem, mp=mp, t2d=text.reshape(R, m.text_dim)))
    for (C, e1, e2), items in by_c.items():
        if GROUPED_SMM and len(items) > 1:
            mems = ops.smm_memproj_compact_grouped([it for _, it in items], eps1=e1, eps2=e2)
        else:
            mems = [ops.smm_memproj_compact(it["feat"], it["ln1_g"], it["ln1_b"], it["gram"], it["hvec"], it["evar"], it["Cm"], eps1=e1, eps2=e2)
                    for _, it in items]
        for (i, _), mem in zip(items, mems):
            st[i]["mem"] = mem

    def fold_weights(s, ca):
        mp, Cm = s["mp"], s["Cm"]
        if s["compact"]:
            return _PREP.get(("xfold", ca, Cm), (mp[1].weight, mp[1].bias, mp[2].weight, mp[2].bias, ca.k_proj.weight, ca.v_proj.weight),
                             lambda: _fold_memory_affine(mp[1], mp[2], ca, Cm))
        return ca.k_proj.weight, wT(ca.v_proj), None

    def self_attn_and_query(sel, xs, li):
        lay = [st[i]["dec"].decoder[li] for i in sel]
        qkv = ops.linear_t_grouped([dict(x=x, wT=_PREP.get(("qkvT", l.self_attn), (l.self_attn.q_proj.weight, l.self_attn.k_proj.weight, l.self_attn.v_proj.weight),
                                                             lambda sa=l.self_attn: torch.cat([sa.q_proj.weight, sa.k_proj.weight, sa.v_proj.weight], 0).detach().t().contiguous()),
                                         ln=(l.norm1.weight, l.norm1.bias, l.norm1.eps)) for x, l in zip(xs, lay)])
        att = ops.attn_tokens_packed_grouped([q.reshape(B, K, 3 * Wd) for q in qkv], heads, lay[0].self_attn.scale)
        xs = ops.linear_t_grouped([dict(x=a.reshape(R, Wd), wT=wT(l.self_attn.proj), bias=l.self_attn.proj.bias, res=x, gscale=branch_gains(l)[0])
                                   for a, l, x in zip(att, lay, xs)])
        qc = ops.linear_t_grouped([dict(x=x, wT=wT(l.cross_attn.q_proj), ln=(l.norm2.weight, l.norm2.bias, l.norm2.eps)) for x, l in zip(xs, lay)])
        qfs, groups = [], []
        for i, q, l in zip(sel, qc, lay):
            Cm = st[i]["Cm"]
            wkf = fold_weights(st[i], l.cross_attn)[0]
            qf = torch.empty((R, heads * Cm), device=dev, dtype=torch.float32)
            qfs.append(qf)
            groups += [dict(x=q[:, h * dh:(h + 1) * dh], wT=wkf[h * dh:(h + 1) * dh], out=qf[:, h * Cm:(h + 1) * Cm]) for h in range(heads)]
        _grouped_chunks(groups)
        return xs, qfs

    def text_prefix(sel):
        x0 = ops.linear_t_grouped([dict(x=st[i]["t2d"], wT=wT(st[i]["dec"].text_proj[1]), bias=st[i]["dec"].text_proj[1].bias,
                                        ln=(st[i]["dec"].text_proj[0].weight, st[i]["dec"].text_proj[0].bias, st[i]["dec"].text_proj[0].eps)) for i in sel])
        x1, qf1 = self_attn_and_query(sel, x0, 0)
        t2v = ops.linear_t_grouped([dict(x=st[i]["t2d"], wT=wT(st[i]["m"].text_to_visual), bias=st[i]["m"].text_to_visual.bias) for i in sel])
        return list(zip(x1, qf1, t2v))

    def prefix_params(s, text):
        dec, m, mp = s["dec"], s["m"], s["mp"]
        l0 = dec.decoder[0]
        return [text, dec.text_proj[0].weight, dec.text_proj[0].bias, dec.text_proj[1].weight, dec.text_proj[1].bias, l0.norm1.weight, l0.norm1.bias,
                l0.self_attn.q_proj.weight, l0.self_attn.k_proj.weight, l0.self_attn.v_proj.weight, l0.self_attn.proj.weight, l0.self_attn.proj.bias,
                l0.norm2.weight, l0.norm2.bias, l0.cross_attn.q_proj.weight, l0.cross_attn.k_proj.weight, mp[1].weight, mp[1].bias, mp[2].weight,
                m.text_to_visual.weight, m.text_to_visual.bias] + ([l0.gamma_sa] if hasattr(l0, "gamma_sa") else [])

    if torch.is_grad_enabled() or not cache_prefix:
        pre = text_prefix(list(range(L)))
    else:
        pre = [None] * L
        todo = []
        for i, (s, text) in enumerate(zip(st, texts)):
            hit = _PREP.peek(("prefix", s["m"], s["Cm"]), prefix_params(s, text))
            if hit is None:
                todo.append(i)
            else:
                pre[i] = hit
        if todo:
            for i, val in zip(todo, text_prefix(todo)):
                pre[i] = _PREP.get(("prefix", st[i]["m"], st[i]["Cm"]), prefix_params(st[i], texts[i]), lambda val=val: val)
    xs = [p[0] for p in pre]
    qfs = [p[1] for p in pre]
    t2vs = [p[2] for p in pre]

    every = list(range(L))
    for li in range(nlayers):
        lay = [s["dec"].decoder[li] for s in st]
        if li > 0:
            xs, qfs = self_attn_and_query(every, xs, li)
        avs, groups = [], []
        assert all(l.cross_attn.scale == lay[0].cross_attn.scale for l in lay)
        if GROUPED_SMM and len(st) > 1:
            os_ = ops.smm_xattn_grouped([qf.reshape(B, K, heads, s["Cm"]) for s, qf in zip(st, qfs)], [s["mem"] for s in st], lay[0].cross_attn.scale)
        else:
            os_ = [ops.smm_xattn(qf.reshape(B, K, heads, s["Cm"]), s["mem"], lay[0].cross_attn.scale) for s, qf in zip(st, qfs)]
        for s, l, o in zip(st, lay, os_):
            Cm, ca = s["Cm"], l.cross_attn
            _, wvf, bvf = fold_weights(s, ca)
            o = o.reshape(R, heads * Cm)
            av = torch.empty((R, Wd), device=dev, dtype=torch.float32)
            avs.append(av)
            groups += [dict(x=o[:, h * Cm:(h + 1) * Cm], wT=wvf[:, h * dh:(h + 1) * dh], bias=None if bvf is None else bvf[h * dh:(h + 1) * dh],
                            out=av[:, h * dh:(h + 1) * dh]) for h in range(heads)]
        _grouped_chunks(groups)
        xs = ops.linear_t_grouped([dict(x=av, wT=wT(l.cross_attn.proj), bias=l.cross_attn.proj.bias, res=x, gscale=branch_gains(l)[1])
                                   for av, l, x in zip(avs, lay, xs)])
        hm = ops.linear_t_grouped([dict(x=x, wT=wT(l.mlp[0]), bias=l.mlp[0].bias, act_out=ops.ACT_GELU, ln=(l.norm3.weight, l.norm3.bias, l.norm3.eps))
                                   for x, l in zip(xs, lay)])
        xs = ops.linear_t_grouped([dict(x=h_, wT=wT(l.mlp[3]), bias=l.mlp[3].bias, res=x, gscale=branch_gains(l)[2]) for h_, l, x in zip(hm, lay, xs)])
    if plain_out:
        return ops.linear_t_grouped([dict(x=x, wT=wT(s["dec"].out_proj[1]), bias=s["dec"].out_proj[1].bias,
                                          ln=(s["dec"].out_proj[0].weight, s["dec"].out_proj[0].bias, s["dec"].out_proj[0].eps)) for x, s in zip(xs, st)])
    return ops.linear_t_grouped([dict(x=x, wT=wT(s["dec"].out_proj[1]), bias=s["dec"].out_proj[1].bias, res=t2v, gscale=s["m"].gamma,
                                      ln=(s["dec"].out_proj[0].weight, s["dec"].out_proj[0].bias, s["dec"].out_proj[0].eps)) for x, s, t2v in zip(xs, st, t2vs)])


def decoder_tokens_flash(m, feat, text, plain_out=False):
    dec = m.context_decoder
    Wd, heads = dec.width, dec.heads
    assert Wd == 256 and heads == 4, "the half-precision cross-attention kernel is built for 4 heads x 64"
    B, C, H, W = feat.shape
    K = text.shape[1]
    R = B * K
    mp = dec.memory_proj
    wmp = _PREP.get(("mp", mp[1]), (mp[1].weight,), lambda: ops.pack_conv_weight(mp[1].weight.detach().reshape(Wd, C, 1, 1).contiguous()))
    mem = ops.smm_memproj(feat, mp[0].weight, mp[0].bias, wmp, mp[1].bias, mp[2].weight, mp[2].bias, eps=mp[0].eps).reshape(B, Wd, H, W)
    t2d = text.reshape(R, m.text_dim)
    x = ops.linear_t(t2d, wT(dec.text_proj[1]), bias=dec.text_proj[1].bias, ln=(dec.text_proj[0].weight, dec.text_proj[0].bias, dec.text_proj[0].eps))
    for l in dec.decoder:
        g_sa, g_ca, g_mlp = branch_gains(l)
        sa, ca = l.self_attn, l.cross_attn
        qkvT = _PREP.get(("qkvT", sa), (sa.q_proj.weight, sa.k_proj.weight, sa.v_proj.weight),
                         lambda sa=sa: torch.cat([sa.q_proj.weight, sa.k_proj.weight, sa.v_proj.weight], 0).detach().t().contiguous())
        qkv = ops.linear_t(x, qkvT, ln=(l.norm1.weight, l.norm1.bias, l.norm1.eps))
        att = ops.attn_tokens_packed_f16(qkv.reshape(B, K, 3 * Wd), heads, sa.scale)
        x = ops.linear_t(att.reshape(R, Wd), wT(sa.proj), bias=sa.proj.bias, res=x, gscale=g_sa)
        qc = ops.linear_t(x, wT(ca.q_proj), ln=(l.norm2.weight, l.norm2.bias, l.norm2.eps))
        wk = _PREP.get(("kconv", ca), (ca.k_proj.weight,), lambda ca=ca: ops.pack_conv_weight(ca.k_proj.weight.detach().reshape(Wd, Wd, 1, 1).contiguous()))
        wv = _PREP.get(("vconv", ca), (ca.v_proj.weight,), lambda ca=ca: ops.pack_conv_weight(ca.v_proj.weight.detach().reshape(Wd, Wd, 1, 1).contiguous()))
        kk = ops.conv2d(mem, wk, None, 1, Wd).reshape(B, Wd, H * W)
        vv = ops.conv2d(mem, wv, None, 1, Wd).reshape(B, Wd, H * W)
        av = ops.smm_xattn_kv_f16(qc.reshape(B, K, Wd), kk, vv, heads, ca.scale)
        x = ops.linear_t(av.reshape(R, Wd), wT(ca.proj), bias=ca.proj.bias, res=x, gscale=g_ca)
        hm = ops.linear_t(x, wT(l.mlp[0]), bias=l.mlp[0].bias, act_out=ops.ACT_GELU, ln=(l.norm3.weight, l.norm3.bias, l.norm3.eps))
        x = ops.linear_t(hm, wT(l.mlp[3]), bias=l.mlp[3].bias, res=x, gscale=g_mlp)
    op = dec.out_proj
    if plain_out:
        return ops.linear_t(x, wT(op[1]), bias=op[1].bias, ln=(op[0].weight, op[0].bias, op[0].eps))
    t2v = ops.linear_t(t2d, wT(m.text_to_visual), bias=m.text_to_visual.bias)
    return ops.linear_t(x, wT(op[1]), bias=op[1].bias, res=t2v, gscale=m.gamma, ln=(op[0].weight, op[0].bias, op[0].eps))


def _scoremaps(feats, tvs, idx):
    ok = all(f.shape[2] * f.shape[3] % 4 == 0 and f.data_ptr() % 16 == 0 and (f.stride(0) % 4 == 0 or f.shape[0] == 1) for f in feats)
    if GROUPED_SMM and ok and 1 < len(feats) <= ops._lib.SCOREMAP_MAX_GROUPS and len({tv.shape[1] for tv in tvs}) == 1:
        return ops.scoremap_grouped(feats, tvs, idx)
    return [ops.scoremap(f, tv, idx) for f, tv in zip(feats, tvs)]


def _grouped_chunks(groups):
    n = ops._lib.LINEAR_MAX_GROUPS
    for i in range(0, len(groups), n):
        ops.linear_t_grouped(groups[i:i + n])


def _fold_memory_affine(lin, ln2, ca, Cm):
    W = lin.weight.detach().double()
    b = lin.bias.detach().double()
    Wd, C = W.shape
    P = torch.zeros((Wd, Cm), dtype=torch.float64, device=W.device)
    P[:, :C] = W - W.mean(dim=0, keepdim=True)
    P[:, C] = b - b.mean()
    P *= ln2.weight.detach().double()[:, None]
    WvT = ca.v_proj.weight.detach().double().t()
    wkf = (ca.k_proj.weight.detach().double() @ P).float().contiguous()
    wvf = (P.t() @ WvT).float().contiguous()
    bvf = (ln2.bias.detach().double() @ WvT).float().contiguous()
    return wkf, wvf, bvf


class ResBlock(nn.Module):
    def __init__(self, dim_in, dim_out, time_dim, groups=8):
        super().__init__()
        self.dim_in, self.dim_out, self.groups = dim_in, dim_out, groups
        self.mlp = nn.Linear(time_dim, dim_out * 2)
        self.conv1 = nn.Conv2d(dim_in, dim_out, 3, padding=1)
        self.norm1 = nn.GroupNorm(groups, dim_out)
        self.conv2 = nn.Conv2d(dim_out, dim_out, 3, padding=1)
        self.norm2 = nn.GroupNorm(groups, dim_out)
        self.res_conv = nn.Conv2d(dim_in, dim_out, 1) if dim_in != dim_out else nn.Identity()

    def run(self, src0, src1, film, vec=None, out=None):
        B, _, H, W = src0.shape
        Co, G, HW = self.dim_out, self.groups, H * W
        h1, ab1 = ops.conv2d(src0, packed(self.conv1), self.conv1.bias, 3, Co, src1=src1,
                             gn=dict(groups=G, gamma=self.norm1.weight, beta=self.norm1.bias, film=film, eps=self.norm1.eps))
        h2, (a2, b2) = ops.conv2d(h1, packed(self.conv2), self.conv2.bias, 3, Co, pro=ab1,
                                  gn=dict(groups=G, gamma=self.norm2.weight, beta=self.norm2.bias, eps=self.norm2.eps))
        if isinstance(self.res_conv, nn.Identity):
            assert src1 is None
            return ops.affine_silu_add(h2, (a2, b2), res=src0, vec=vec, out=out)
        return ops.conv2d(src0, packed(self.res_conv), self.res_conv.bias, 1, Co, src1=src1, aux=(h2, a2, b2), vec=vec, out=out)


class ChanLayerNorm(nn.Module):
    def __init__(self, dim):
        super().__init__()
        self.weight = nn.Parameter(torch.ones(dim))
        self.bias = nn.Parameter(torch.zeros(dim))


class CrossAttention(nn.Module):

    def __init__(self, dim, ctx_dim, num_heads=4):
        super().__init__()
        self.dim, self.num_heads = dim, num_heads
        self.scale = (dim // num_heads) ** -0.5
        self.norm = ChanLayerNorm(dim)
        self.q_proj = nn.Conv2d(dim, dim, 1, bias=False)
        self.k_proj = nn.Linear(ctx_dim, dim, bias=False)
        self.v_proj = nn.Linear(ctx_dim, dim, bias=False)
        self.proj = nn.Conv2d(dim, dim, 1)

    def single_token_vec(self, ctx):
        B = ctx.shape[0]
        v = ops.linear(ctx.reshape(B, -1), self.v_proj.weight)
        return ops.linear(v, self.proj.weight.reshape(self.dim, self.dim), self.proj.bias)

    def run(self, x, ctx, out=None):
        B, C, H, W = x.shape
        M = ctx.shape[1]
        xn = ops.chan_layernorm(x, self.norm.weight, self.norm.bias)
        q = ops.conv2d(xn, packed(self.q_proj), None, 1, C)
        c2 = ctx.reshape(B * M, -1)
        k = ops.linear(c2, self.k_proj.weight).reshape(B, M, C)
        v = ops.linear(c2, self.v_proj.weight).reshape(B, M, C)
        o = ops.attn_ctx(q, k, v, self.num_heads, self.scale)
        return ops.conv2d(o, packed(self.proj), self.proj.bias, 1, C, res=x, out=out)


class SelfAttention(nn.Module):
    def __init__(self, dim, num_heads=4):
        super().__init__()
        self.dim, self.num_heads = dim, num_heads
        self.scale = (dim // num_heads) ** -0.5
        self.norm = ChanLayerNorm(dim)
        self.qkv = nn.Conv2d(dim, dim * 3, 1, bias=False)
        self.proj = nn.Conv2d(dim, dim, 1)

    def run(self, x, vec=None):
        xn = ops.chan_layernorm(x, self.norm.weight, self.norm.bias)
        qkv = ops.conv2d(xn, packed(self.qkv), None, 1, 3 * self.dim)
        o = ops.attn_self(qkv, self.num_heads, self.scale)
        return ops.conv2d(o, packed(self.proj), self.proj.bias, 1, self.dim, res=x, vec=vec)


class Downsample(nn.Module):
    def __init__(self, dim_in, dim_out):
        super().__init__()
        self.dim_out = dim_out
        self.conv = nn.Conv2d(dim_in * 4, dim_out, 1)

    def run(self, x):
        return ops.conv2d(x, packed(self.conv), self.conv.bias, 1, self.dim_out, mode=ops.CONV_UNSHUFFLE2)


class Upsample(nn.Module):
    def __init__(self, dim_in, dim_out):
        super().__init__()
        self.dim_out = dim_out
        self.conv = nn.Conv2d(dim_in, dim_out, 3, padding=1)

    def run(self, x):
        return ops.conv2d(x, packed(self.conv), self.conv.bias, 3, self.dim_out, mode=ops.CONV_UPSAMPLE2)


class SameConv(nn.Module):
    def __init__(self, dim_in, dim_out):
        super().__init__()
        self.dim_out = dim_out
        self.conv = nn.Conv2d(dim_in, dim_out, 3, padding=1)

    def run(self, x):
        return ops.conv2d(x, packed(self.conv), self.conv.bias, 3, self.dim_out)


class Level(nn.Module):
    pass


class LearnableForwardUNet_MultiScoreMap(nn.Module):

    def __init__(self, in_nc=2, out_nc=5, nf=64, ch_mult=(1, 2, 4, 4), context_dim=512, text_module="scoremap", score_map_chan=16,
                 if_MultiScoreMap=True, score_map_ch_mult=(1, 1, 2, 4), score_map_ngf=16, use_image_context=False,
                 use_degra_context=False, CLIP_ScoreMapModule=None, artifact_types=ARTIFACT_TYPES, gn_groups=8, attn_heads=4,
                 **_ignored):
        super().__init__()
        if use_degra_context:
            raise NotImplementedError("use_degra_context=True is outside the hot-path scope (config.yml:133 sets it False)")
        self.text_module = text_module
        self.use_image_context = use_image_context
        self.type_map_ind = {n: i for i, n in enumerate(artifact_types)}
        self.depth = len(ch_mult)
        self.nf, self.out_nc, self.in_nc = nf, out_nc, in_nc
        K = len(artifact_types)
        time_dim = nf * 4
        self.time_dim = time_dim
        mult = [1] + list(ch_mult)
        self.init_conv = nn.Conv2d(in_nc, nf, 7, padding=3)
        self.time_mlp = nn.Sequential(nn.Linear(nf, time_dim), nn.GELU(), nn.Linear(time_dim, time_dim))
        half = nf // 2
        self.register_buffer("time_freqs", torch.exp(torch.arange(half, dtype=torch.float32) * (-math.log(10000.0) / (half - 1))),
                             persistent=False)
        use_sm = text_module == "scoremap"
        self.CLIP_ScoreMapModule = CLIP_ScoreMapModule if use_sm else None
        self.n_sm = (self.depth if if_MultiScoreMap else 1) if use_sm else 0
        self.downs = nn.ModuleList()
        self.ups = nn.ModuleList()
        self.sm_embed = nn.ModuleList()
        self.level_dims = []
        for i in range(self.depth):
            din, dout = nf * mult[i], nf * mult[i + 1]
            smc = (score_map_ngf * score_map_ch_mult[i] if if_MultiScoreMap else score_map_chan) if i < self.n_sm else 0
            self.level_dims.append((din, dout, smc))
            lv = Level()
            lv.res1 = ResBlock(din, din, time_dim, gn_groups)
            lv.res2 = ResBlock(din, din, time_dim, gn_groups)
            if use_image_context:
                lv.ca1 = CrossAttention(din, context_dim, attn_heads)
                lv.ca2 = CrossAttention(din, context_dim, attn_heads)
            lv.down = Downsample(din, dout) if i != self.depth - 1 else SameConv(din, dout)
            self.downs.append(lv)
            if i < self.n_sm:
                self.sm_embed.append(nn.Conv2d(K, smc, 3, padding=1))
            up = Level()
            up.res1 = ResBlock(dout + din + smc, dout, time_dim, gn_groups)
            up.res2 = ResBlock(dout + din, dout, time_dim, gn_groups)
            if use_image_context:
                up.ca1 = CrossAttention(dout, context_dim, attn_heads)
                up.ca2 = CrossAttention(dout, context_dim, attn_heads)
            up.up = Upsample(dout, din) if i != 0 else SameConv(dout, din)
            self.ups.insert(0, up)
        mid = nf * mult[-1]
        self.mid_res1 = ResBlock(mid, mid, time_dim, gn_groups)
        self.mid_attn = SelfAttention(mid, attn_heads)
        if use_image_context:
            self.mid_ca = CrossAttention(mid, context_dim, attn_heads)
        self.mid_res2 = ResBlock(mid, mid, time_dim, gn_groups)
        self.final_res = ResBlock(nf * 2, nf, time_dim, gn_groups)
        self.final_conv = nn.Conv2d(nf, out_nc, 3, padding=1)
        self._ctx_cache = None
        self._idx_cache = {}

    def score_map_modules(self):
        m = self.CLIP_ScoreMapModule
        if m is None:
            return []
        return list(m) if isinstance(m, (nn.ModuleList, list, tuple)) else [m]

    def resblocks(self):
        rbs = []
        for lv in self.downs:
            rbs += [lv.res1, lv.res2]
        rbs += [self.mid_res1, self.mid_res2]
        for up in self.ups:
            rbs += [up.res1, up.res2]
        rbs.append(self.final_res)
        return rbs

    def cross_attns(self):
        if not self.use_image_context:
            return []
        cas = []
        for lv in self.downs:
            cas += [lv.ca1, lv.ca2]
        cas.append(self.mid_ca)
        for up in self.ups:
            cas += [up.ca1, up.ca2]
        return cas

    def class_index(self, names, device):
        if torch.is_tensor(names):
            if names.dtype != torch.int32 or names.dim() != 1 or names.device.type != torch.device(device).type:
                raise ValueError(f"class_index: an index tensor must be int32 [B] on {device}, got {names.dtype} {tuple(names.shape)} on {names.device}")
            return names
        key = (tuple(names), str(device))
        hit = self._idx_cache.get(key)
        if hit is None:
            hit = torch.tensor([self.type_map_ind[n] for n in names], dtype=torch.int32, device=device)
            self._idx_cache[key] = hit
        return hit

    def held_cache_values(self):
        held = []
        for mod in self.modules():
            slot = _PREP.store.get(mod)
            if slot:
                held.extend(slot.values())
        held.extend(m._text_cache for m in self.score_map_modules() if m._text_cache is not None)
        if self._ctx_cache is not None:
            held.append(self._ctx_cache[1])
        held.extend(self._idx_cache.values())
        return held

    def _films(self, temb):
        rbs = self.resblocks()
        w, b = _PREP.get(("film", self), [p for rb in rbs for p in (rb.mlp.weight, rb.mlp.bias)],
                         lambda: (torch.cat([rb.mlp.weight for rb in rbs], 0).detach().contiguous(),
                                  torch.cat([rb.mlp.bias for rb in rbs], 0).detach().contiguous()))
        allf = ops.linear(temb, w, b, act_in=ops.ACT_SILU)
        out, o = {}, 0
        for rb in rbs:
            out[id(rb)] = allf[:, o:o + 2 * rb.dim_out]
            o += 2 * rb.dim_out
        return out

    def _ctx_vecs(self, ctx):
        cas = self.cross_attns()
        key = (ctx._version, tuple(ctx.shape), _weight_epoch()) + tuple((p.data_ptr(), p._version) for ca in cas
                                                        for p in (ca.v_proj.weight, ca.proj.weight, ca.proj.bias))
        c = self._ctx_cache
        if c is not None and c[0] == key and c[2]() is ctx:
            return c[1]
        vecs = {id(ca): ca.single_token_vec(ctx) for ca in cas}
        self._ctx_cache = (key, vecs, weakref.ref(ctx))
        return vecs

    def forward(self, x_a, x_b, t, names, text_encoder, image_context=None):
        if torch.is_grad_enabled() and any(p.requires_grad for p in self.parameters()):
            from .unet_autograd import forward_train
            return forward_train(self, x_a, x_b, t, names, text_encoder, image_context)
        return self.forward_infer(x_a, x_b, t, names, text_encoder, image_context)

    conv_dtype = "f32"

    @torch.no_grad()
    def forward_infer(self, x_a, x_b, t, names, text_encoder, image_context=None):
        with ops.conv_operands(self.conv_dtype):
            return self._forward_infer(x_a, x_b, t, names, text_encoder, image_context)

    def _forward_infer(self, x_a, x_b, t, names, text_encoder, image_context=None):
        dev = x_a.device
        B, _, H, W = x_a.shape
        if not torch.is_tensor(t):
            t = torch.full((B,), float(t), dtype=torch.float32, device=dev)
        t = t.reshape(-1).to(device=dev, dtype=torch.float32)
        if t.numel() == 1 and B > 1:
            t = t.expand(B)
        t = t.contiguous()
        idx = self.class_index(names, dev)
        ctx = image_context if self.use_image_context else None
        single = ctx is not None and ctx.shape[1] == 1
        general = ctx is not None and not single
        if ctx is not None:
            ctx = ctx.contiguous()
        vecs = self._ctx_vecs(ctx) if single else {}

        def ca_vec(ca_name, holder):
            return vecs[id(getattr(holder, ca_name))] if single else None

        if self.nf == 64 and self.time_dim == 256:
            temb = ops.time_mlp(t, self.time_freqs, self.time_mlp[0].weight, self.time_mlp[0].bias, self.time_mlp[2].weight, self.time_mlp[2].bias)
        else:
            temb = ops.linear(ops.linear(ops.time_embed(t, self.nf, self.time_freqs), self.time_mlp[0].weight, self.time_mlp[0].bias, act_out=ops.ACT_GELU),
                              self.time_mlp[2].weight, self.time_mlp[2].bias)
        films = self._films(temb)

        x = ops.conv2d(x_a, packed(self.init_conv), self.init_conv.bias, 7, self.nf, src1=x_b)
        x_ = x
        hs, sms = [], []
        use_sm = self.CLIP_ScoreMapModule is not None
        sm_feats, sm_skips = [], []
        for i, lv in enumerate(self.downs):
            din, dout, smc = self.level_dims[i]
            Hi, Wi = x.shape[2], x.shape[3]
            x = lv.res1.run(x, None, films[id(lv.res1)], vec=ca_vec("ca1", lv))
            if general:
                x = lv.ca1.run(x, ctx)
            hs.append(x)
            use_sm = i < self.n_sm
            if use_sm:
                skip = torch.empty((B, din + smc, Hi, Wi), device=dev, dtype=torch.float32)
                xo = skip[:, :din]
            else:
                skip, xo = None, None
            x = lv.res2.run(x, None, films[id(lv.res2)], vec=ca_vec("ca2", lv), out=None if general else xo)
            if general:
                x = lv.ca2.run(x, ctx, out=xo)
            if use_sm:
                sm_feats.append(x)
                sm_skips.append(skip)
                hs.append(skip)
            else:
                hs.append(x)
            x = lv.down.run(x)
        side = cur = None
        if self.n_sm > 0:
            def smm_phase():
                smms = self.score_map_modules()
                texts = [m.text_embeddings(text_encoder, B) for m in smms]
                tvs = decoder_tokens_grouped(smms, sm_feats, texts)
                scores = _scoremaps(sm_feats, [tv.reshape(B, m.n_cls, feat.shape[1]) for m, feat, tv in zip(smms, sm_feats, tvs)], idx)
                for i, ((score, sel), skip) in enumerate(zip(scores, sm_skips)):
                    din, dout, smc = self.level_dims[i]
                    ops.conv2d(score, packed(self.sm_embed[i]), self.sm_embed[i].bias, 3, smc, out=skip[:, din:])
                    sms.append(sel)
            if SMM_SIDE and x.is_cuda:
                if getattr(self, "_side_stream", None) is None:
                    self._side_stream = torch.cuda.Stream()
                side, cur = self._side_stream, torch.cuda.current_stream()
                side.wait_stream(cur)
                with torch.cuda.stream(side):
                    smm_phase()
                for sel in sms:
                    sel.record_stream(cur)
            else:
                smm_phase()
        x = self.mid_res1.run(x, None, films[id(self.mid_res1)])
        x = self.mid_attn.run(x, vec=ca_vec("mid_ca", self))
        if general:
            x = self.mid_ca.run(x, ctx)
        x = self.mid_res2.run(x, None, films[id(self.mid_res2)])
        if side is not None:
            side.wait_stream(cur)
            for t in [x, x_] + hs:
                t.record_stream(side)
            with torch.cuda.stream(side):
                pred = self._decode(x, x_, hs, films, vecs if single else None, general, ctx, idx)
            pred.record_stream(cur)
            return (pred, sms) if self.text_module == "scoremap" else pred
        return self._decode(x, x_, hs, films, vecs if single else None, general, ctx, idx, sms if self.text_module == "scoremap" else None)

    def _decode(self, x, x_, hs, films, vecs, general, ctx, idx, sms=None):
        def ca_vec(ca_name, holder):
            return vecs[id(getattr(holder, ca_name))] if vecs is not None else None
        for up in self.ups:
            x = up.res1.run(x, hs.pop(), films[id(up.res1)], vec=ca_vec("ca1", up))
            if general:
                x = up.ca1.run(x, ctx)
            x = up.res2.run(x, hs.pop(), films[id(up.res2)], vec=ca_vec("ca2", up))
            if general:
                x = up.ca2.run(x, ctx)
            x = up.up.run(x)
        x = self.final_res.run(x, x_, films[id(self.final_res)])
        pred = ops.conv3x3_select(x, self.final_conv.weight.detach(), self.final_conv.bias, idx)
        if self.text_module == "scoremap" and sms is not None:
            return pred, sms
        return pred
```

### instancediff_amd/ops.py

```python
import contextlib
import ctypes as C
import math
import os
import threading

import torch

from . import _lib
from ._lib import ConvDesc, check

CONV_NORMAL, CONV_UPSAMPLE2, CONV_UNSHUFFLE2 = 0, 1, 2
ACT_NONE, ACT_SILU, ACT_GELU = 0, 1, 2
SDE_STEP, SDE_MEAN, SDE_ODE = 0, 1, 2

PROFILE = None
ALGO_TRACE = None
WGRAD_TRACE = None


def launch_count():
    return int(_lib.load().idiff_launch_count())


def _stream():
    return C.c_void_p(torch.cuda.current_stream().cuda_stream)


def _p(t):
    return None if t is None else C.c_void_p(t.data_ptr())


def _chk(t, name="tensor", dtype=torch.float32):
    if t is None:
        return
    if not t.is_cuda:
        raise _lib.IdiffError(f"{name} must live on the GPU (the hot path has no CPU fallback)")
    if t.dtype != dtype:
        raise _lib.IdiffError(f"{name} must be {dtype}, got {t.dtype}")


def _bs(t, name="tensor"):
    _chk(t, name)
    exp = 1
    for d in range(t.dim() - 1, 0, -1):
        if t.shape[d] != 1 and t.stride(d) != exp:
            raise _lib.IdiffError(f"{name}: samples must be contiguous (shape {tuple(t.shape)}, strides {t.stride()})")
        exp *= t.shape[d]
    return t.stride(0) if t.shape[0] > 1 else max(exp, t.stride(0))


def _c(t, name="tensor", dtype=torch.float32):
    _chk(t, name, dtype)
    if t is not None and not t.is_contiguous():
        raise _lib.IdiffError(f"{name} must be contiguous")
    return t


WINOGRAD = bool(int(os.environ.get("IDIFF_WINOGRAD", "1")))
X3 = bool(int(os.environ.get("IDIFF_X3", "1")))
WINOGRAD4 = WINOGRAD and bool(int(os.environ.get("IDIFF_WINOGRAD4", "1")))
WINOGRAD4_DGRAD = bool(int(os.environ.get("IDIFF_WINOGRAD4_DGRAD", "1")))


CONV_ALGO_DIRECT, CONV_ALGO_WINOGRAD, CONV_ALGO_STREAM1X1, CONV_ALGO_WINOGRAD4, CONV_ALGO_WINOGRAD4H, CONV_ALGO_X3 = 0, 1, 2, 3, 4, 5
CONV_ALGO_BF16 = 6
_ALGO_REQUEST = threading.local()
CONV_OPERANDS = ("f32", "bf16")
_OPERANDS = threading.local()


@contextlib.contextmanager
def conv_operands(kind):
    if kind not in CONV_OPERANDS:
        raise ValueError(f"conv operands must be one of {CONV_OPERANDS}, got {kind!r}")
    old = getattr(_OPERANDS, "kind", "f32")
    _OPERANDS.kind = kind
    try:
        yield
    finally:
        _OPERANDS.kind = old


def current_conv_operands():
    return getattr(_OPERANDS, "kind", "f32")


@contextlib.contextmanager
def request_conv3x3_algo(algo):
    old = getattr(_ALGO_REQUEST, "algo", None)
    _ALGO_REQUEST.algo = algo
    try:
        yield
    finally:
        _ALGO_REQUEST.algo = old


def _alloc_conv_images(w, transpose, bf16=False):
    lib = _lib.load()
    _c(w, "weight")
    co, ci, k, _ = w.shape
    out = torch.empty((k * k, co, ci) if transpose else (k * k, ci, co), device=w.device, dtype=torch.float32)
    if bf16 and k == 3:
        out.bf16 = torch.empty((lib.idiff_conv_weight_bf16_bytes(co, ci, 1 if transpose else 0) // 2,), device=w.device, dtype=torch.int16)
    if k == 3 and WINOGRAD and co % 8 == 0 and ci % 8 == 0 and (ci if transpose else co) % 16 == 0:
        cconv, kconv = (ci, co) if transpose else (co, ci)
        out.wino = torch.empty((16 * kconv * ((cconv + 63) // 64) * 64,), device=w.device, dtype=torch.float32)
        if WINOGRAD4 and (WINOGRAD4_DGRAD or not transpose):
            out.wino4 = torch.empty((36 * kconv * ((cconv + 63) // 64) * 64,), device=w.device, dtype=torch.float32)
    cconv1, kconv1 = (ci, co) if transpose else (co, ci)
    if k == 1 and X3 and cconv1 % 64 == 0 and kconv1 >= 32 and kconv1 % 8 == 0:
        out.x3 = torch.empty((lib.idiff_conv1x1_x3_image_bytes(cconv1, kconv1) // 2,), device=w.device, dtype=torch.int16)
    return out


def _fill_conv_images(out, w, transpose, algo=None):
    lib = _lib.load()
    co, ci, k, _ = w.shape
    tr = 1 if transpose else 0
    if algo is None or algo == CONV_ALGO_DIRECT:
        fn = lib.idiff_pack_conv_weight_T if transpose else lib.idiff_pack_conv_weight
        check(fn(_p(w), _p(out), co, ci, k, _stream()), "pack_conv_weight")
    if hasattr(out, "wino") and (algo is None or algo == CONV_ALGO_WINOGRAD):
        check(lib.idiff_pack_conv_weight_wino(_p(w), _p(out.wino), co, ci, tr, _stream()), "pack_conv_weight_wino")
    if hasattr(out, "wino4") and (algo is None or algo in (CONV_ALGO_WINOGRAD4, CONV_ALGO_WINOGRAD4H)):
        check(lib.idiff_pack_conv_weight_wino4(_p(w), _p(out.wino4), co, ci, tr, _stream()), "pack_conv_weight_wino4")
    if hasattr(out, "x3") and (algo is None or algo == CONV_ALGO_X3):
        cconv1, kconv1 = (ci, co) if transpose else (co, ci)
        wm = w.reshape(co, ci).t().contiguous() if transpose else w
        check(lib.idiff_pack_conv1x1_x3(_p(wm), out.x3.data_ptr(), cconv1, kconv1, _stream()), "pack_conv1x1_x3")
    if hasattr(out, "bf16") and (algo is None or algo == CONV_ALGO_BF16):
        check(lib.idiff_pack_conv_weight_bf16(_p(w), out.bf16.data_ptr(), co, ci, tr, _stream()), "pack_conv_weight_bf16")


def pack_conv_weight(w, transpose=False, bf16=False):
    out = _alloc_conv_images(w, transpose, bf16)
    _fill_conv_images(out, w, transpose)
    return out


class LazyConvWeight:

    def __init__(self, w, transpose=False):
        self.w, self.transpose = _c(w, "weight"), transpose


def conv2d(src0, wpk, bias, ks, Cout, src1=None, mode=CONV_NORMAL, pro=None, out=None, res=None, vec=None, aux=None,
           want_stats=False, algo=None, gn=None, operands=None):
    lib = _lib.load()
    B, C0, Hin, Win = src0.shape
    operands = current_conv_operands() if operands is None else operands
    if operands not in CONV_OPERANDS:
        raise ValueError(f"conv operands must be one of {CONV_OPERANDS}, got {operands!r}")
    bf16 = operands == "bf16" and ks == 3
    lazy = wpk if isinstance(wpk, LazyConvWeight) else None
    if lazy is not None:
        wpk = _alloc_conv_images(lazy.w, lazy.transpose, bf16 or algo == CONV_ALGO_BF16)
    d = ConvDesc()
    if bf16:
        d.operands = 1
    wb = getattr(wpk, "bf16", None)
    if wb is not None and ks == 3:
        d.wbf16 = wb.data_ptr()
    if algo is not None:
        d.algo_request = 1 + algo
    elif ks == 3 and getattr(_ALGO_REQUEST, "algo", None) is not None:
        d.algo_request = -(1 + _ALGO_REQUEST.algo)
    d.src0, d.src0_bstride, d.C0 = src0.data_ptr(), _bs(src0, "src0"), C0
    if src1 is not None:
        assert src1.shape[0] == B and src1.shape[2:] == src0.shape[2:]
        d.src1, d.src1_bstride, d.C1 = src1.data_ptr(), _bs(src1, "src1"), src1.shape[1]
    d.B, d.Hin, d.Win, d.mode, d.ks, d.Cout = B, Hin, Win, mode, ks, Cout
    _c(wpk, "wpk")
    d.wpk = wpk.data_ptr()
    wino = getattr(wpk, "wino", None)
    if wino is not None and ks == 3:
        d.wwino = wino.data_ptr()
        wino4 = getattr(wpk, "wino4", None)
        if wino4 is not None:
            d.wwino4 = wino4.data_ptr()
    x3 = getattr(wpk, "x3", None)
    if x3 is not None and ks == 1 and mode in (CONV_NORMAL, CONV_UNSHUFFLE2):
        d.wx3 = x3.data_ptr()
    if bias is not None:
        d.bias = _c(bias, "bias").data_ptr()
    if pro is not None:
        d.pro_a, d.pro_b = _c(pro[0], "pro_a").data_ptr(), _c(pro[1], "pro_b").data_ptr()
    if mode == CONV_UPSAMPLE2:
        Hout, Wout = Hin * 2, Win * 2
    elif mode == CONV_UNSHUFFLE2:
        Hout, Wout = Hin // 2, Win // 2
    else:
        Hout, Wout = Hin, Win
    if out is None:
        out = torch.empty((B, Cout, Hout, Wout), device=src0.device, dtype=torch.float32)
    else:
        assert tuple(out.shape) == (B, Cout, Hout, Wout), (out.shape, (B, Cout, Hout, Wout))
    d.out, d.out_bstride = out.data_ptr(), _bs(out, "out")
    if res is not None:
        assert res.shape == out.shape
        d.res, d.res_bstride = res.data_ptr(), _bs(res, "res")
    if vec is not None:
        assert tuple(vec.shape) == (B, Cout)
        d.vec = _c(vec, "vec").data_ptr()
    if aux is not None:
        t, a, b = aux
        assert t.shape == out.shape
        d.aux, d.aux_bstride = t.data_ptr(), _bs(t, "aux")
        d.aux_a, d.aux_b = _c(a, "aux_a").data_ptr(), _c(b, "aux_b").data_ptr()
    stats = None
    bufs = gn.get("bufs") if gn is not None else None
    if want_stats or gn is not None:
        nt = lib.idiff_conv2d_num_tiles(Hout, Wout)
        stats = bufs[0] if bufs is not None else torch.empty((B, nt, Cout, 2), device=src0.device, dtype=torch.float32)
        assert tuple(stats.shape) == (B, nt, Cout, 2) and stats.is_contiguous() and stats.dtype == torch.float32
        d.stats = stats.data_ptr()
    gn_out = None
    if gn is not None:
        if bufs is not None:
            ga, gb = bufs[1], bufs[2]
            assert tuple(ga.shape) == (B, Cout) == tuple(gb.shape) and ga.is_contiguous() and gb.is_contiguous()
        else:
            ga, gb = torch.empty((B, Cout), device=src0.device, dtype=torch.float32), torch.empty((B, Cout), device=src0.device, dtype=torch.float32)
        d.gn_groups, d.gn_eps = int(gn["groups"]), float(gn.get("eps", 1e-5))
        d.gn_gamma, d.gn_beta = _c(gn["gamma"], "gn gamma").data_ptr(), _c(gn["beta"], "gn beta").data_ptr()
        film = gn.get("film")
        if film is not None:
            _chk(film, "film")
            assert film.shape[0] == B and film.shape[1] == 2 * Cout and film.stride(1) == 1
            d.gn_film, d.gn_film_ld = film.data_ptr(), film.stride(0)
        d.gn_out_a, d.gn_out_b = ga.data_ptr(), gb.data_ptr()
        gn_out = (ga, gb)
        if gn.get("want_mean_rstd"):
            mr = bufs[3] if bufs is not None else torch.empty((B, d.gn_groups, 2), device=src0.device, dtype=torch.float32)
            assert tuple(mr.shape) == (B, d.gn_groups, 2) and mr.is_contiguous()
            d.gn_mean_rstd = mr.data_ptr()
            gn_out = (ga, gb, mr)
    planned = None
    if lazy is not None:
        planned = lib.idiff_conv2d_plan(C.byref(d))
        check(min(planned, 0), "conv2d_plan")
        _fill_conv_images(wpk, lazy.w, lazy.transpose, planned)
    if PROFILE is not None:
        e0, e1 = torch.cuda.Event(enable_timing=True), torch.cuda.Event(enable_timing=True)
        e0.record()
        check(lib.idiff_conv2d_fwd(C.byref(d), _stream()), "conv2d_fwd")
        e1.record()
        Cin = (C0 * 4 if mode == CONV_UNSHUFFLE2 else C0) + (src1.shape[1] if src1 is not None else 0)
        PROFILE.append(dict(ks=ks, mode=mode, Cin=Cin, Cout=Cout, B=B, Hout=Hout, Wout=Wout, e0=e0, e1=e1, algo=lib.idiff_conv2d_last_algo(),
                            flops=2.0 * Cin * Cout * ks * ks * Hout * Wout * B))
    else:
        check(lib.idiff_conv2d_fwd(C.byref(d), _stream()), "conv2d_fwd")
    if planned is not None and lib.idiff_conv2d_last_algo() != planned:
        raise RuntimeError("conv2d: planned kernel %d, launched %d" % (planned, lib.idiff_conv2d_last_algo()))
    if ALGO_TRACE is not None:
        Cin = (C0 * 4 if mode == CONV_UNSHUFFLE2 else C0) + (src1.shape[1] if src1 is not None else 0)
        ALGO_TRACE[(lib.idiff_conv2d_last_algo(), ks, Cin, Cout, Hout, Wout)] += 1
    if gn is not None:
        return (out, gn_out, stats) if want_stats else (out, gn_out)
    return (out, stats) if want_stats else out


def gn_finalize(stats, groups, HW, gamma, beta, film=None, eps=1e-5, want_mean_rstd=False):
    lib = _lib.load()
    B, nt, Cc, _ = stats.shape
    a = torch.empty((B, Cc), device=stats.device, dtype=torch.float32)
    b = torch.empty_like(a)
    mr = torch.empty((B, groups, 2), device=stats.device, dtype=torch.float32) if want_mean_rstd else None
    film_ld = 0
    if film is not None:
        _chk(film, "film")
        assert film.shape[0] == B and film.shape[1] == 2 * Cc and film.stride(1) == 1
        film_ld = film.stride(0)
    check(lib.idiff_gn_finalize(_p(_c(stats)), nt, B, Cc, groups, HW, _p(_c(gamma)), _p(_c(beta)), _p(film), film_ld, eps,
                                _p(a), _p(b), _p(mr), _stream()), "gn_finalize")
    return (a, b, mr) if want_mean_rstd else (a, b)


def affine_silu_add(h, ab=None, res=None, vec=None, out=None):
    lib = _lib.load()
    B, Cc = h.shape[:2]
    HW = h.shape[2] * h.shape[3]
    if out is None:
        out = torch.empty(h.shape, device=h.device, dtype=torch.float32)
    a, b = ab if ab is not None else (None, None)
    check(lib.idiff_affine_silu_add(_p(h), _bs(h, "h"), _p(_c(a)), _p(_c(b)), _p(res), _bs(res, "res") if res is not None else 0,
                                    _p(_c(vec)), _p(out), _bs(out, "out"), B, Cc, HW, _stream()), "affine_silu_add")
    return out


def linear(x, w, bias=None, res=None, gscale=None, act_in=ACT_NONE, act_out=ACT_NONE, out=None):
    lib = _lib.load()
    _chk(x, "x"), _chk(w, "w")
    assert x.dim() == 2 and w.dim() == 2 and x.stride(1) == 1 and w.stride(1) == 1 and x.shape[1] == w.shape[1]
    R, K = x.shape
    N = w.shape[0]
    if out is None:
        out = torch.empty((R, N), device=x.device, dtype=torch.float32)
    assert out.stride(1) == 1 and tuple(out.shape) == (R, N)
    if res is not None:
        assert res.stride(1) == 1 and tuple(res.shape) == (R, N)
    check(lib.idiff_linear_fwd(_p(x), x.stride(0), _p(w), w.stride(0), _p(_c(bias)), _p(res), res.stride(0) if res is not None else 0,
                               _p(_c(gscale)), _p(out), out.stride(0), R, K, N, act_in, act_out, _stream()), "linear_fwd")
    return out


def linear_t(x, wT, bias=None, res=None, gscale=None, act_in=ACT_NONE, act_out=ACT_NONE, out=None, ln=None):
    lib = _lib.load()
    _chk(x, "x"), _chk(wT, "wT")
    assert x.dim() == 2 and wT.dim() == 2 and x.stride(1) == 1 and wT.stride(1) == 1 and x.shape[1] == wT.shape[0]
    R, K = x.shape
    N = wT.shape[1]
    if out is None:
        out = torch.empty((R, N), device=x.device, dtype=torch.float32)
    assert out.stride(1) == 1 and tuple(out.shape) == (R, N)
    if res is not None:
        assert res.stride(1) == 1 and tuple(res.shape) == (R, N)
    if ln is not None:
        assert act_in == ACT_NONE
        check(lib.idiff_linear_t_ln_fwd(_p(x), x.stride(0), _p(_c(ln[0])), _p(_c(ln[1])), float(ln[2]), _p(wT), wT.stride(0), _p(_c(bias)), _p(res),
                                        res.stride(0) if res is not None else 0, _p(_c(gscale)), _p(out), out.stride(0), R, K, N, act_out,
                                        _stream()), "linear_t_ln_fwd")
        return out
    check(lib.idiff_linear_t_fwd(_p(x), x.stride(0), _p(wT), wT.stride(0), _p(_c(bias)), _p(res), res.stride(0) if res is not None else 0,
                                 _p(_c(gscale)), _p(out), out.stride(0), R, K, N, act_in, act_out, _stream()), "linear_t_fwd")
    return out


def linear_t_grouped(groups):
    lib = _lib.load()
    n = len(groups)
    assert 1 <= n <= _lib.LINEAR_MAX_GROUPS, n
    arr = (_lib.LinearGroup * n)()
    outs = []
    for d, g in zip(arr, groups):
        x, wT = g["x"], g["wT"]
        _chk(x, "x"), _chk(wT, "wT")
        assert x.dim() == 2 and wT.dim() == 2 and x.stride(1) == 1 and wT.stride(1) == 1 and x.shape[1] == wT.shape[0]
        R, K = x.shape
        N = wT.shape[1]
        out = g.get("out")
        if out is None:
            out = torch.empty((R, N), device=x.device, dtype=torch.float32)
        assert out.stride(1) == 1 and tuple(out.shape) == (R, N)
        res, bias, gs, ln = g.get("res"), g.get("bias"), g.get("gscale"), g.get("ln")
        d.x, d.ldx, d.wT, d.ldw = x.data_ptr(), x.stride(0), wT.data_ptr(), wT.stride(0)
        d.bias = _c(bias, "bias").data_ptr() if bias is not None else None
        if res is not None:
            assert res.stride(1) == 1 and tuple(res.shape) == (R, N)
            d.res, d.ldr = res.data_ptr(), res.stride(0)
        d.gscale = _c(gs, "gscale").data_ptr() if gs is not None else None
        d.out, d.ldo = out.data_ptr(), out.stride(0)
        if ln is not None:
            assert g.get("act_in", ACT_NONE) == ACT_NONE
            d.ln_g, d.ln_b, d.ln_eps = _c(ln[0], "ln_g").data_ptr(), _c(ln[1], "ln_b").data_ptr(), float(ln[2])
        d.R, d.K, d.N, d.act_in, d.act_out = R, K, N, g.get("act_in", ACT_NONE), g.get("act_out", ACT_NONE)
        outs.append(out)
    check(lib.idiff_linear_t_grouped_fwd(arr, n, _stream()), "linear_t_grouped_fwd")
    return outs


def attn_tokens_packed_grouped(qkvs, heads, scale):
    lib = _lib.load()
    n = len(qkvs)
    assert 1 <= n <= _lib.LINEAR_MAX_GROUPS
    B, Nq, C3 = qkvs[0].shape
    Cc = C3 // 3
    PA = C.c_void_p * n
    q, k, v, o = PA(), PA(), PA(), PA()
    outs = []
    for i, t in enumerate(qkvs):
        _c(t, "qkv")
        assert tuple(t.shape) == (B, Nq, C3)
        out = torch.empty((B, Nq, Cc), device=t.device, dtype=torch.float32)
        base = t.data_ptr()
        q[i], k[i], v[i], o[i] = base, base + 4 * Cc, base + 8 * Cc, out.data_ptr()
        outs.append(out)
    check(lib.idiff_attn_tokens_grouped_fwd(q, k, v, o, n, B, Nq, Nq, Cc, heads, scale, C3, C3, _stream()), "attn_tokens_grouped_fwd")
    return outs


def linear_t_heads(x, wT, bias, out, heads, K, N, x_hs, w_hs, b_hs, o_hs):
    lib = _lib.load()
    _chk(x, "x"), _chk(wT, "wT"), _chk(out, "out")
    assert x.dim() == 2 and wT.dim() == 2 and out.dim() == 2 and x.stride(1) == 1 and wT.stride(1) == 1 and out.stride(1) == 1
    R = x.shape[0]
    assert out.shape[0] == R and (heads - 1) * x_hs + K <= x.shape[1] and (heads - 1) * o_hs + N <= out.shape[1]
    assert (heads - 1) * w_hs + (K - 1) * wT.stride(0) + N <= wT.numel()
    check(lib.idiff_linear_t_heads_fwd(_p(x), x.stride(0), x_hs, _p(wT), wT.stride(0), w_hs, _p(_c(bias)), b_hs, _p(out), out.stride(0), o_hs,
                                       R, K, N, heads, _stream()), "linear_t_heads_fwd")
    return out


def smm_memproj(feat, ln1_g, ln1_b, wpk, bias, ln2_g, ln2_b, eps=1e-5):
    lib = _lib.load()
    B, Cc, H, W = feat.shape
    out = torch.empty((B, 256, H * W), device=feat.device, dtype=torch.float32)
    check(lib.idiff_smm_memproj_fwd(_p(feat), _bs(feat, "feat"), _p(_c(ln1_g)), _p(_c(ln1_b)), _p(_c(wpk)), _p(_c(bias)), _p(_c(ln2_g)),
                                    _p(_c(ln2_b)), _p(out), B, Cc, H * W, eps, _stream()), "smm_memproj_fwd")
    return out


def smm_memproj_compact(feat, ln1_g, ln1_b, gram, hvec, evar, Cm, eps1=1e-5, eps2=1e-5):
    lib = _lib.load()
    B, Cc, H, W = feat.shape
    out = torch.empty((B, Cm, H * W), device=feat.device, dtype=torch.float32)
    check(lib.idiff_smm_memproj_compact_fwd(_p(feat), _bs(feat, "feat"), _p(_c(ln1_g)), _p(_c(ln1_b)), _p(_c(gram)), _p(_c(hvec)), float(evar),
                                            _p(out), B, Cc, H * W, Cm, eps1, eps2, _stream()), "smm_memproj_compact_fwd")
    return out


def memory_variance_form(lin_weight, lin_bias):
    W = lin_weight.detach().double()
    b = lin_bias.detach().double()
    Wc = W - W.mean(dim=0, keepdim=True)
    bc = b - b.mean()
    n = W.shape[0]
    return (Wc.t() @ Wc / n).float().contiguous(), (Wc.t() @ bc / n).float().contiguous(), float(bc.dot(bc) / n)


def layernorm_rows(x, gamma, beta, eps=1e-5, want_mean_rstd=False):
    lib = _lib.load()
    _chk(x, "x")
    assert x.dim() == 2 and x.stride(1) == 1
    R, Cc = x.shape
    out = torch.empty((R, Cc), device=x.device, dtype=torch.float32)
    mr = torch.empty((R, 2), device=x.device, dtype=torch.float32) if want_mean_rstd else None
    check(lib.idiff_layernorm_rows_fwd(_p(x), x.stride(0), _p(_c(gamma)), _p(_c(beta)), _p(out), Cc, R, Cc, eps, _p(mr), _stream()),
          "layernorm_rows")
    return (out, mr) if want_mean_rstd else out


def time_embed(t, dim, freqs=None):
    lib = _lib.load()
    _c(t, "t"), _c(freqs, "freqs")
    B = t.numel()
    out = torch.empty((B, dim), device=t.device, dtype=torch.float32)
    check(lib.idiff_time_embed_fwd(_p(t), _p(freqs), B, dim, _p(out), _stream()), "time_embed")
    return out


def chan_layernorm(x, gamma, beta, eps=1e-5, want_mean_rstd=False):
    lib = _lib.load()
    B, Cc, H, W = x.shape
    out = torch.empty((B, Cc, H, W), device=x.device, dtype=torch.float32)
    mr = torch.empty((B, H * W, 2), device=x.device, dtype=torch.float32) if want_mean_rstd else None
    check(lib.idiff_chan_layernorm_fwd(_p(x), _bs(x, "x"), _p(_c(gamma)), _p(_c(beta)), _p(out), Cc * H * W, B, Cc, H * W, eps, _p(mr),
                                       _stream()), "chan_layernorm")
    return (out, mr) if want_mean_rstd else out


ATTN_DTYPE = os.environ.get("IDIFF_ATTN_DTYPE", "f32").lower()


def attn_self(qkv, heads, scale, want_lse=False):
    lib = _lib.load()
    _c(qkv, "qkv")
    B, C3, H, W = qkv.shape
    Cc, N = C3 // 3, H * W
    out = torch.empty((B, Cc, H, W), device=qkv.device, dtype=torch.float32)
    if ATTN_DTYPE in ("bf16", "f16") and not want_lse and Cc // heads == 64 and N % 4 == 0:
        fn = lib.idiff_attn_self_bf16_fwd if ATTN_DTYPE == "bf16" else lib.idiff_attn_self_f16_fwd
        check(fn(_p(qkv), _p(out), B, Cc, N, heads, scale, _stream()), "attn_self_%s_fwd" % ATTN_DTYPE)
        return out
    lse = torch.empty((B, heads, N), device=qkv.device, dtype=torch.float32) if want_lse else None
    check(lib.idiff_attn_self_fwd(_p(qkv), _p(out), _p(lse), B, Cc, N, heads, scale, _stream()), "attn_self_fwd")
    return (out, lse) if want_lse else out


def attn_ctx(q, k, v, heads, scale):
    lib = _lib.load()
    _c(q, "q"), _c(k, "k"), _c(v, "v")
    B, Cc, H, W = q.shape
    M = k.shape[1]
    out = torch.empty_like(q)
    check(lib.idiff_attn_ctx_fwd(_p(q), _p(k), _p(v), _p(out), B, Cc, H * W, M, heads, scale, _stream()), "attn_ctx_fwd")
    return out


def attn_tokens(q, k, v, heads, scale):
    lib = _lib.load()
    _c(q, "q"), _c(k, "k"), _c(v, "v")
    B, Nq, Cc = q.shape
# ... 526 lines not shown
```

Baseline: 44.14 steps/s.

## Add sub-pixel Winograd F(5x5,2x2) kernel for upsample-2x 3x3 convolutions

Adds a dedicated kernel for the nearest-upsample 3x3 convolution. It folds the upsample into four 2x2 sub-pixel phase kernels and runs them with a Winograd F(5x5,2x2) transform on the low-resolution input, so the upsampled tensor is never convolved directly and the redundant taps are skipped. It includes a new weight-image packer, LDS-DMA double-buffered pipelining in a persistent grid, and auto-selection for large problems (Cin*Cout*H*W >= 1e8). The cost is a large amount of hand-written inline-asm code, extra weight memory, and possible fp32 numerical differences from the larger Winograd tile.

```diff
diff --git a/include/idiff.h b/include/idiff.h
--- a/include/idiff.h
+++ b/include/idiff.h
@@ -48,6 +48,7 @@
     float* stats;
     const float* wwino;
     const float* wwino4;
+    const float* wwino4u;
     const float* gn_gamma;
     const float* gn_beta;
     const float* gn_film;
@@ -72,6 +73,7 @@
 #define IDIFF_CONV_ALGO_WINOGRAD4H 4
 #define IDIFF_CONV_ALGO_X3 5
 #define IDIFF_CONV_ALGO_BF16 6
+#define IDIFF_CONV_ALGO_WINOGRAD4U 7
 int idiff_conv2d_last_algo(void);
 int idiff_conv2d_plan(const idiff_conv_desc* d);
 long long idiff_conv1x1_x3_image_bytes(int Cout, int Cin);
@@ -80,6 +82,7 @@
 int idiff_pack_conv_weight_T(const float* w, float* wpk, int Cout, int Cin, int ks, idiff_stream_t stream);
 int idiff_pack_conv_weight_wino(const float* w, float* wwino, int Cout, int Cin, int transpose, idiff_stream_t stream);
 int idiff_pack_conv_weight_wino4(const float* w, float* wwino4, int Cout, int Cin, int transpose, idiff_stream_t stream);
+int idiff_pack_conv_weight_wino4u(const float* w, float* wwino4u, int Cout, int Cin, idiff_stream_t stream);
 long long idiff_conv_weight_bf16_bytes(int Cout, int Cin, int transpose);
 int idiff_pack_conv_weight_bf16(const float* w, void* image, int Cout, int Cin, int transpose, idiff_stream_t stream);
 
diff --git a/instancediff_amd/_lib.py b/instancediff_amd/_lib.py
--- a/instancediff_amd/_lib.py
+++ b/instancediff_amd/_lib.py
@@ -26,6 +26,7 @@
         ("stats", C.c_void_p),
         ("wwino", C.c_void_p),
         ("wwino4", C.c_void_p),
+        ("wwino4u", C.c_void_p),
         ("gn_gamma", C.c_void_p), ("gn_beta", C.c_void_p), ("gn_film", C.c_void_p), ("gn_film_ld", C.c_int64), ("gn_eps", C.c_float),
         ("gn_groups", C.c_int32), ("gn_out_a", C.c_void_p), ("gn_out_b", C.c_void_p), ("gn_mean_rstd", C.c_void_p),
         ("algo_request", C.c_int32),
@@ -71,6 +72,7 @@
     "idiff_pack_conv_weight_T": (I, [P, P, I, I, I, c_stream]),
     "idiff_pack_conv_weight_wino": (I, [P, P, I, I, I, c_stream]),
     "idiff_pack_conv_weight_wino4": (I, [P, P, I, I, I, c_stream]),
+    "idiff_pack_conv_weight_wino4u": (I, [P, P, I, I, c_stream]),
     "idiff_conv_weight_bf16_bytes": (C.c_longlong, [I, I, I]),
     "idiff_pack_conv_weight_bf16": (I, [P, P, I, I, I, c_stream]),
     "idiff_conv1x1_x3_image_bytes": (C.c_longlong, [I, I]),
diff --git a/instancediff_amd/csrc/conv_args.h b/instancediff_amd/csrc/conv_args.h
--- a/instancediff_amd/csrc/conv_args.h
+++ b/instancediff_amd/csrc/conv_args.h
@@ -67,6 +67,9 @@
 int launch_conv_wino4(const ConvArgs& a, int mode, hipStream_t st);
 int launch_conv_wino4h(const ConvArgs& a, int mode, hipStream_t st);
 
+long long conv_wino4u_items(const ConvArgs& a, int ks, int mode, const float* wimg);
+int launch_conv_wino4u(const ConvArgs& a, const float* wimg, hipStream_t st);
+
 bool conv1x1_x3_eligible(const ConvArgs& a, int mode);
 int launch_conv1x1_x3(const ConvArgs& a, int mode, const void* wx3, hipStream_t st);
 
diff --git a/instancediff_amd/csrc/conv_igemm.hip b/instancediff_amd/csrc/conv_igemm.hip
--- a/instancediff_amd/csrc/conv_igemm.hip
+++ b/instancediff_amd/csrc/conv_igemm.hip
@@ -619,7 +619,8 @@
     const bool hard = d->algo_request > 0;
     const int req = (hard ? d->algo_request : -d->algo_request) - 1;
     IDIFF_CHECK_ARG(req == -1 || req == IDIFF_CONV_ALGO_DIRECT || req == IDIFF_CONV_ALGO_WINOGRAD || req == IDIFF_CONV_ALGO_WINOGRAD4 ||
-                        req == IDIFF_CONV_ALGO_WINOGRAD4H || req == IDIFF_CONV_ALGO_X3 || req == IDIFF_CONV_ALGO_BF16,
+                        req == IDIFF_CONV_ALGO_WINOGRAD4H || req == IDIFF_CONV_ALGO_X3 || req == IDIFF_CONV_ALGO_BF16 ||
+                        (hard && req == IDIFF_CONV_ALGO_WINOGRAD4U),
                     "conv2d: bad algo_request %d", d->algo_request);
     IDIFF_CHECK_ARG(d->operands == 0 || d->operands == 1, "conv2d: bad operands %d", d->operands);
     {
@@ -655,6 +656,13 @@
             return take(IDIFF_CONV_ALGO_X3);
         }
     }
+    {
+        const bool requ = req == IDIFF_CONV_ALGO_WINOGRAD4U;
+        const bool can = d->operands == 0 && idiff_detail::conv_wino4u_items(a, d->ks, d->mode, d->wwino4u) > 0;
+        IDIFF_CHECK_ARG(!(hard && requ) || can, "conv2d: bad algo_request %d: the sub-pixel F(5x5,2x2) form takes a single-source fp32 upsample 3x3 "
+                        "with a bias at most (Cin %% 8, Cin >= 16, Cout %% 16) and a sub-pixel image", d->algo_request);
+        if (can && (requ || (req == -1 && (long long)a.Cin * a.Cout * a.Hin * a.Win >= 100000000ll))) return take(IDIFF_CONV_ALGO_WINOGRAD4U);
+    }
     static const int w4h_mode = [] {
         const char* e = getenv("IDIFF_W4H");
         return e ? atoi(e) : 1;
@@ -690,6 +698,7 @@
     switch (p.algo) {
         case IDIFF_CONV_ALGO_X3: return idiff_detail::launch_conv1x1_x3(a, d->mode, d->wx3, st);
         case IDIFF_CONV_ALGO_BF16: rc = idiff_detail::launch_conv_bf16(a, d->mode, d->wbf16, st); break;
+        case IDIFF_CONV_ALGO_WINOGRAD4U: return idiff_detail::launch_conv_wino4u(a, d->wwino4u, st);
         case IDIFF_CONV_ALGO_WINOGRAD4H: rc = idiff_detail::launch_conv_wino4h(a, d->mode, st); break;
         case IDIFF_CONV_ALGO_WINOGRAD4: rc = idiff_detail::launch_conv_wino4(a, d->mode, st); break;
         case IDIFF_CONV_ALGO_WINOGRAD: rc = idiff_detail::launch_conv_wino(a, d->mode, st); break;
diff --git a/instancediff_amd/csrc/conv_wino4u.hip b/instancediff_amd/csrc/conv_wino4u.hip
--- /dev/null
+++ b/instancediff_amd/csrc/conv_wino4u.hip
@@ -0,0 +1,550 @@
+#include "conv_args.h"
+#include "wino_common.h"
+
+using idiff_detail::ConvArgs;
+
+namespace {
+
+using namespace idiff_wino;
+
+constexpr int CK = 4;
+constexpr int NTILE = 32;
+constexpr int RS = 170;
+constexpr int PS = 6 * RS;
+
+constexpr int PSD = 1040;
+constexpr int MAXQ = RS - 161;
+constexpr int NT = 512;
+constexpr int NL = 8;
+constexpr int R_FLOATS = 4 * PSD;
+constexpr int V_FLOATS = 9 * 2 * 64 * 4;
+constexpr int U_FLOATS = 9 * 4 * 64 * 4;
+
+struct Geo4u {
+    int ncobv;
+    int nruns;
+    int tiles_x, tiles_y;
+    int total;
+};
+
+template <bool HEAVY>
+__device__ __forceinline__ void conv_wino4u_body(const ConvArgs& a, const Geo4u& g, const float* const wimg, float* smem) {
+    float* const Rb = smem;
+    float* const Vb = smem + 2 * R_FLOATS;
+    float* const Ub = Vb + 2 * V_FLOATS;
+    float* const econst = Ub + 2 * U_FLOATS;
+    int* const gtab = reinterpret_cast<int*>(econst + 128);
+    constexpr unsigned R_BYTES = R_FLOATS * 4, U_BYTES = U_FLOATS * 4;
+    const unsigned lds_base = __builtin_amdgcn_readfirstlane((unsigned)reinterpret_cast<unsigned long long>(smem));
+    const unsigned U_LDS0 = lds_base + (2 * R_FLOATS + 2 * V_FLOATS) * 4;
+
+    const int tid = threadIdx.x;
+    const int lane = tid & 63;
+    const int wave = __builtin_amdgcn_readfirstlane(tid >> 6);
+    const int k4 = lane >> 4;
+    const int cb = wave & 3;
+    const int tblk = wave >> 2;
+    const int HWin = a.Hin * a.Win;
+    const int nchunks = a.Cin / CK;
+
+    constexpr int RSRC_FLAGS = 0x00020000;
+    struct View {
+        int b, vcb, t0;
+    };
+    const float *p0A = a.src0, *puA = wimg, *p0B = a.src0, *puB = wimg;
+    View vA = {0, 0, 0}, vB = {0, 0, 0};
+    int nrB = 0;
+    int it_b = 0, it_cob = 0, it_run = 0;
+    int d_cob, d_run, d_b;
+    {
+        const int G0 = gridDim.x;
+        d_cob = G0 % g.ncobv;
+        const int r1 = G0 / g.ncobv;
+        d_run = r1 % g.nruns;
+        d_b = r1 / g.nruns;
+    }
+    auto decode_first = [&](int item) {
+        it_cob = item % g.ncobv;
+        const int r1 = item / g.ncobv;
+        it_run = r1 % g.nruns;
+        it_b = r1 / g.nruns;
+    };
+    auto advance_item = [&]() {
+        it_cob += d_cob;
+        int carry = it_cob >= g.ncobv;
+        it_cob -= carry ? g.ncobv : 0;
+        it_run += d_run + carry;
+        carry = it_run >= g.nruns;
+        it_run -= carry ? g.nruns : 0;
+        it_b += d_b + carry;
+    };
+    auto decode_B = [&]() {
+        vB.b = it_b, vB.vcb = it_cob, vB.t0 = it_run * NTILE;
+        puB = scalar_ptr(wimg + (long long)it_cob * U_FLOATS);
+        p0B = scalar_ptr(a.src0 + (long long)it_b * a.bs0);
+        nrB = 0x7fffffff;
+    };
+    const int trole = wave & 1;
+    const int thalf = (wave >> 1) & 1;
+    const int jtr = 16 * thalf + (lane & 15);
+    auto tile_col = [&](const View& v) {
+        const int tx0 = v.t0 % g.tiles_x;
+        const int q = (tx0 + jtr) / g.tiles_x;
+        return 5 * jtr + (q < MAXQ ? q : MAXQ);
+    };
+    auto write_table = [&](const View& v) {
+        int t = tid;
+        asm volatile("" : "+v"(t));
+        const int ty0 = v.t0 / g.tiles_x, tx0 = v.t0 - ty0 * g.tiles_x;
+        const int len0 = g.tiles_x - tx0 < NTILE ? g.tiles_x - tx0 : NTILE;
+        const int L0 = 5 * len0 + 1, LW = 5 * g.tiles_x + 1;
+#pragma unroll
+        for (int i = 0; i < NL; ++i) {
+            const int e = t + i * NT;
+            const int ci = e >> 10, rem = e & 1023;
+            const int r = rem / RS, c = rem - r * RS;
+            int q, off, jb, txs;
+            if (c < L0) {
+                q = 0, off = c, jb = 0, txs = tx0;
+            } else {
+                const int c1 = c - L0;
+                const int s = c1 / LW;
+                q = 1 + s, off = c1 - s * LW, jb = len0 + s * g.tiles_x, txs = 0;
+            }
+            const int jc = jb + (off > 0 ? (off - 1) / 5 : 0);
+            const int iy = 5 * (ty0 + q) - 1 + r, ix = 5 * txs - 1 + off;
+            const bool in = rem < PS && jc < NTILE && q <= MAXQ && ty0 + q < g.tiles_y && (unsigned)iy < (unsigned)a.Hin && (unsigned)ix < (unsigned)a.Win;
+            gtab[i * NT + tid] = in ? (ci * HWin + iy * a.Win + ix) * 4 : -1;
+        }
+    };
+    int tcA = 0, tcB = 0;
+    auto shift_B_to_A = [&]() { p0A = p0B, puA = puB, vA = vB, tcA = tcB; };
+    const int ustride_b = g.ncobv * U_FLOATS * 4;
+
+    const unsigned u_voff = tid * 16;
+    auto dma_u = [&](int p, int buf) {
+        const bool inA = p < nchunks;
+        const int so = (inA ? p : p - nchunks) * ustride_b;
+        const __amdgpu_buffer_rsrc_t rsu = __builtin_amdgcn_make_buffer_rsrc(const_cast<float*>(inA ? puA : puB), 0, inA ? 0x7fffffff : nrB, RSRC_FLAGS);
+        const unsigned lds0 = __builtin_amdgcn_readfirstlane(U_LDS0 + (unsigned)buf * U_BYTES + (unsigned)wave * 1024u);
+        asm volatile(
+            "s_nop 4\n\ts_mov_b32 m0, %2\n\ts_nop 0\n\tbuffer_load_dwordx4 %0, %1, %3 offen lds\n\t"
+            "s_add_u32 m0, m0, 0x2000\n\ts_nop 0\n\tbuffer_load_dwordx4 %0, %1, %4 offen lds\n\t"
+            "s_add_u32 m0, m0, 0x2000\n\ts_nop 0\n\tbuffer_load_dwordx4 %0, %1, %5 offen lds\n\t"
+            "s_add_u32 m0, m0, 0x2000\n\ts_nop 0\n\tbuffer_load_dwordx4 %0, %1, %6 offen lds"
+            ::"v"(u_voff), "s"(rsu), "s"(lds0), "s"(so), "s"(so + NT * 16), "s"(so + 2 * NT * 16), "s"(so + 3 * NT * 16)
+            : "memory", "scc");
+        if (!HEAVY) {
+            const unsigned lds4 = __builtin_amdgcn_readfirstlane(lds0 + 4 * NT * 16 - 256 * 16);
+            asm volatile("s_nop 4\n\ts_mov_b32 m0, %2\n\ts_nop 0\n\tbuffer_load_dwordx4 %0, %1, %3 offen lds" ::"v"(u_voff), "s"(rsu), "s"(lds4),
+                         "s"(so + 4 * NT * 16 - 256 * 16)
+                         : "memory");
+        }
+    };
+    auto dma_u_piece = [&](int p, int buf, int i) {
+        const bool inA = p < nchunks;
+        const int so = (inA ? p : p - nchunks) * ustride_b + (i < 4 ? i * NT * 16 : 4 * NT * 16 - 256 * 16);
+        const __amdgpu_buffer_rsrc_t rsu = __builtin_amdgcn_make_buffer_rsrc(const_cast<float*>(inA ? puA : puB), 0, inA ? 0x7fffffff : nrB, RSRC_FLAGS);
+        const unsigned lds0 = __builtin_amdgcn_readfirstlane(U_LDS0 + (unsigned)buf * U_BYTES + (unsigned)wave * 1024u + (unsigned)(i < 4 ? i * NT * 16 : 4 * NT * 16 - 256 * 16));
+        asm volatile("s_nop 4\n\ts_mov_b32 m0, %2\n\ts_nop 0\n\tbuffer_load_dwordx4 %0, %1, %3 offen lds" ::"v"(u_voff), "s"(rsu), "s"(lds0), "s"(so) : "memory");
+    };
+    float rinA[NL], rinB[NL];
+    auto ld_raw = [&](float (&dst)[NL], int p, int i, int goff_i) {
+        const bool inA = p < nchunks;
+        const int so = (inA ? p : p - nchunks) * CK * HWin * 4;
+        const __amdgpu_buffer_rsrc_t rs = __builtin_amdgcn_make_buffer_rsrc(const_cast<float*>(inA ? p0A : p0B), 0, inA ? 0x7fffffff : nrB, RSRC_FLAGS);
+        asm volatile("s_nop 4\n\tbuffer_load_dword %0, %1, %2, %3 offen" : "=v"(dst[i]) : "v"(goff_i), "s"(rs), "s"(so) : "memory");
+    };
+    auto stage = [&](const float (&src)[NL], unsigned rslot, int i0, int i1) {
+        float* const R = reinterpret_cast<float*>(reinterpret_cast<char*>(Rb) + rslot) + tid;
+#pragma unroll
+        for (int i = 0; i < NL; ++i) {
+            if (i < i0 || i >= i1) continue;
+            R[(i >> 1) * PSD + (i & 1) * NT] = src[i];
+        }
+    };
+    constexpr int N_U = HEAVY ? 4 : 5;
+
+    constexpr bool heavy = HEAVY;
+    const float al = trole ? -1.f : -4.f, be = trole ? 2.f : 1.f;
+    const float* const trbase = Rb + k4 * PSD + (heavy ? 1 : trole) * RS;
+    const int ufirst = heavy ? 1 + 2 * trole : 5 * trole;
+    float* const vwbase = Vb + thalf * 256 + lane * 4;
+    float ta[6], tb[6], tlo[6], thi[6];
+    auto rd_row = [&](const float* p, float (&d)[6]) {
+#pragma unroll
+        for (int c = 0; c < 6; ++c) d[c] = p[c];
+    };
+    auto tr_piece = [&](int piece, unsigned rslot, int tc, int buf) {
+        const float* p = reinterpret_cast<const float*>(reinterpret_cast<const char*>(trbase) + rslot) + tc;
+        if (piece == 0) {
+            if (heavy) rd_row(p + 1 * RS, ta), rd_row(p + 3 * RS, tb);
+            else rd_row(p, ta), rd_row(p + 2 * RS, tb);
+        } else if (piece == 1) {
+            if (heavy) {
+#pragma unroll
+                for (int c = 0; c < 6; ++c) tlo[c] = __builtin_fmaf(al, ta[c], tb[c]);
+                rd_row(p, ta), rd_row(p + 2 * RS, tb);
+            } else {
+#pragma unroll
+                for (int c = 0; c < 6; ++c) tlo[c] = __builtin_fmaf(4.f, ta[c], -5.f * tb[c]);
+                rd_row(p + 4 * RS, ta);
+            }
+        } else if (piece == 2) {
+            if (heavy) {
+#pragma unroll
+                for (int c = 0; c < 6; ++c) {
+                    const float X = tlo[c], Y = __builtin_fmaf(al, ta[c], tb[c]);
+                    tlo[c] = __builtin_fmaf(be, Y, X);
+                    thi[c] = __builtin_fmaf(-be, Y, X);
+                }
+            } else {
+#pragma unroll
+                for (int c = 0; c < 6; ++c) tlo[c] += ta[c];
+            }
+        } else {
+            const int which = piece - 3;
+            if (which == 1 && !heavy) return;
+            float o[6];
+            bt6(which ? thi : tlo, o);
+            const int u = ufirst + which;
+            float* const V = vwbase + buf * V_FLOATS;
+            *reinterpret_cast<floatx4*>(V + PF(u) * 512) = floatx4{o[0], o[1], o[2], o[3]};
+            typedef float floatx2 __attribute__((ext_vector_type(2)));
+            *reinterpret_cast<floatx2*>(V + PH(u) * 512 + 2 * (u & 1)) = floatx2{o[4], o[5]};
+        }
+    };
+
+    const int G = gridDim.x;
+    const int first = (int)xcd_remap(blockIdx.x, G);
+    const int last = g.total;
+    if (first >= last) return;
+    auto fetch_bias = [&](const View& v) {
+        float e = 0.f;
+        const int co = (v.vcb >> 1) * 32 + tid;
+        if (tid < 32 && a.bias && co < a.Cout) e = a.bias[co];
+        return e;
+    };
+
+    decode_first(first);
+    decode_B();
+    tcB = tile_col(vB);
+    shift_B_to_A();
+    write_table(vA);
+    if (first + G < last) {
+        advance_item();
+        decode_B();
+        tcB = tile_col(vB);
+    } else {
+        nrB = 0, vB = vA, tcB = tcA;
+    }
+    {
+        const float e0 = fetch_bias(vA);
+        if (tid < 32) econst[tid] = e0;
+    }
+    dma_u(0, 0);
+    {
+        int goff[NL];
+#pragma unroll
+        for (int i = 0; i < NL; ++i) goff[i] = gtab[i * NT + tid];
+#pragma unroll
+        for (int i = 0; i < NL; ++i) ld_raw(rinA, 0, i, goff[i]);
+#pragma unroll
+        for (int i = 0; i < NL; ++i) ld_raw(rinB, 1, i, goff[i]);
+        asm volatile("s_waitcnt vmcnt(0)" : "+v"(rinA[0]), "+v"(rinA[1]), "+v"(rinA[2]), "+v"(rinA[3]), "+v"(rinA[4]), "+v"(rinA[5]), "+v"(rinA[6]), "+v"(rinA[7]),
+                     "+v"(rinB[0]), "+v"(rinB[1]), "+v"(rinB[2]), "+v"(rinB[3]), "+v"(rinB[4]), "+v"(rinB[5]), "+v"(rinB[6]), "+v"(rinB[7])::"memory");
+        stage(rinA, 0 * R_BYTES, 0, NL);
+        stage(rinB, 1 * R_BYTES, 0, NL);
+#pragma unroll
+        for (int i = 0; i < NL; ++i) ld_raw(rinA, 2, i, goff[i]);
+        __syncthreads();
+    }
+#pragma unroll
+    for (int piece = 0; piece < 5; ++piece) tr_piece(piece, 0 * R_BYTES, tcA, 0);
+    asm volatile("s_waitcnt vmcnt(0)" : "+v"(rinA[0]), "+v"(rinA[1]), "+v"(rinA[2]), "+v"(rinA[3]), "+v"(rinA[4]), "+v"(rinA[5]), "+v"(rinA[6]), "+v"(rinA[7])::"memory");
+    __syncthreads();
+    dma_u(1, 1);
+
+    unsigned r_t = 1 * R_BYTES, r_a = 0 * R_BYTES;
+    int epar = 0;
+    for (int item = first; item < last; item += G) {
+        floatx4 acc[36];
+        {
+            const int opoff = lane * 4;
+            floatx4 ob[2], oa[2];
+            ob[0] = *reinterpret_cast<const floatx4*>(Vb + tblk * 256 + opoff);
+            oa[0] = *reinterpret_cast<const floatx4*>(Ub + cb * 256 + opoff);
+            auto chunk = [&](int cc, auto par_tag, auto zero_tag) {
+                constexpr int PAR = decltype(par_tag)::value;
+                constexpr bool ZERO = decltype(zero_tag)::value;
+                const float* V = Vb + PAR * V_FLOATS + tblk * 256 + opoff;
+                const float* U = Ub + PAR * U_FLOATS + cb * 256 + opoff;
+                const float* Vn = Vb + (PAR ^ 1) * V_FLOATS + tblk * 256 + opoff;
+                const float* Un = Ub + (PAR ^ 1) * U_FLOATS + cb * 256 + opoff;
+                int goff[NL];
+                if (cc + 3 == nchunks) write_table(vB);
+#pragma unroll
+                for (int i = 0; i < NL; ++i) goff[i] = gtab[i * NT + tid];
+                float(&rin_s)[NL] = PAR ? rinB : rinA;
+                float(&rin_l)[NL] = PAR ? rinA : rinB;
+                const int tc = cc + 1 < nchunks ? tcA : tcB;
+#pragma unroll
+                for (int q = 0; q < 9; ++q) {
+                    if (q + 1 < 9) {
+                        ob[(q + 1 + PAR) & 1] = *reinterpret_cast<const floatx4*>(V + (q + 1) * 512);
+                        oa[(q + 1 + PAR) & 1] = *reinterpret_cast<const floatx4*>(U + (q + 1) * 1024);
+                    } else {
+                        asm volatile("s_waitcnt vmcnt(%0)" ::"n"(NL) : "memory");
+                        __builtin_amdgcn_sched_barrier(0);
+                        __syncthreads();
+                        if (cc + 1 == nchunks) dma_u(cc + 2, PAR);
+                        else dma_u_piece(cc + 2, PAR, 0);
+                        ob[PAR ^ 1] = *reinterpret_cast<const floatx4*>(Vn);
+                        oa[PAR ^ 1] = *reinterpret_cast<const floatx4*>(Un);
+                    }
+                    const floatx4 bv = ob[(q + PAR) & 1], av = oa[(q + PAR) & 1];
+                    const floatx4 z4 = floatx4{0.f, 0.f, 0.f, 0.f};
+                    acc[4 * q + 0] = __builtin_amdgcn_mfma_f32_16x16x4f32(av.x, bv.x, ZERO ? z4 : acc[4 * q + 0], 0, 0, 0);
+                    acc[4 * q + 1] = __builtin_amdgcn_mfma_f32_16x16x4f32(av.y, bv.y, ZERO ? z4 : acc[4 * q + 1], 0, 0, 0);
+                    acc[4 * q + 2] = __builtin_amdgcn_mfma_f32_16x16x4f32(av.z, bv.z, ZERO ? z4 : acc[4 * q + 2], 0, 0, 0);
+                    acc[4 * q + 3] = __builtin_amdgcn_mfma_f32_16x16x4f32(av.w, bv.w, ZERO ? z4 : acc[4 * q + 3], 0, 0, 0);
+                    if (!ZERO) {
+                        if (q < 3) dma_u_piece(cc + 1, PAR ^ 1, q + 1);
+                        if (q == 3 && !HEAVY) dma_u_piece(cc + 1, PAR ^ 1, 4);
+                    }
+                    if (q == 5) {
+                        asm volatile("s_waitcnt vmcnt(%8)" : "+v"(rin_s[0]), "+v"(rin_s[1]), "+v"(rin_s[2]), "+v"(rin_s[3]), "+v"(rin_s[4]), "+v"(rin_s[5]), "+v"(rin_s[6]), "+v"(rin_s[7]) : "n"(N_U + 2) : "memory");
+                        stage(rin_s, r_a, 0, 3);
+                    }
+                    if (q == 6) stage(rin_s, r_a, 3, 6);
+                    if (q == 7) stage(rin_s, r_a, 6, 8);
+                    auto req = [&](int i) { ld_raw(rin_l, cc + 3, i, goff[i]); };
+                    if (HEAVY && q == 3) req(0);
+                    if (!HEAVY && q == 4) req(0);
+                    if (q == 4) req(1);
+                    if (q == 5) req(2), req(3);
+                    if (q == 6) req(4), req(5);
+                    if (q == 7) req(6), req(7);
+                    if (q < 5) tr_piece(q, r_t, tc, PAR ^ 1);
+                    __builtin_amdgcn_sched_barrier(0);
+                }
+                const unsigned t = r_t;
+                r_t = r_a, r_a = t;
+            };
+            chunk(0, std::integral_constant<int, 0>{}, std::true_type{});
+            chunk(1, std::integral_constant<int, 1>{}, std::false_type{});
+            for (int cc = 2; cc < nchunks; cc += 2) {
+                chunk(cc, std::integral_constant<int, 0>{}, std::false_type{});
+                chunk(cc + 1, std::integral_constant<int, 1>{}, std::false_type{});
+            }
+        }
+
+        const View v = vA;
+        const float* const ebase_item = econst + epar * 64;
+        const bool more = item + G < last;
+        float pre_e = 0.f;
+        if (more) {
+            shift_B_to_A();
+            if (item + 2 * G < last) {
+                advance_item();
+                decode_B();
+                tcB = tile_col(vB);
+            } else {
+                nrB = 0, vB = vA, tcB = tcA;
+            }
+            pre_e = fetch_bias(vA);
+        }
+
+        {
+            int lane_e = lane;
+            asm volatile("" : "+v"(lane_e));
+            const int j = lane_e & 15, k4e = lane_e >> 4;
+            const int HWo = a.Hout * a.Wout;
+            const int py = v.vcb & 1;
+            const int co0 = (v.vcb >> 1) * 32 + cb * 8;
+            const bool wave_live = co0 < a.Cout;
+            const __amdgpu_buffer_rsrc_t rso = __builtin_amdgcn_make_buffer_rsrc(const_cast<float*>(scalar_ptr(a.out + (long long)v.b * a.obs + (long long)co0 * HWo)), 0, wave_live ? HWo * 32 : 0, RSRC_FLAGS);
+            const unsigned ch_off = (unsigned)(2 * k4e) * (unsigned)HWo;
+            const float* const ebase = ebase_item + cb * 8 + 2 * k4e;
+            float zz[6][4][5];
+#pragma unroll
+            for (int u = 0; u < 6; ++u) {
+#pragma unroll
+                for (int r = 0; r < 4; ++r) {
+                    at6_5(acc[pos(u, 0)][r], acc[pos(u, 1)][r], acc[pos(u, 2)][r], acc[pos(u, 3)][r], acc[pos(u, 4)][r], acc[pos(u, 5)][r], zz[u][r]);
+                    asm volatile("" : "+v"(zz[u][r][0]), "+v"(zz[u][r][1]), "+v"(zz[u][r][2]), "+v"(zz[u][r][3]), "+v"(zz[u][r][4]));
+                }
+                __builtin_amdgcn_sched_barrier(0);
+            }
+            constexpr int GS = 164;
+            float* const sb = k4e < 2 ? Vb + V_FLOATS + (wave * 2 + k4e) * GS : reinterpret_cast<float*>(reinterpret_cast<char*>(Rb) + r_a) + (wave * 2 + k4e - 2) * GS;
+            int eoff[12], erow[12];
+#pragma unroll
+            for (int i = 0; i < 6; ++i) {
+#pragma unroll
+                for (int h = 0; h < 2; ++h) {
+                    const int L = 2 * (16 * i + j) + h;
+                    const int jj = (L - 1) / 10, c = (L - 1) - 10 * jj;
+                    const int t = v.t0 + 16 * tblk + jj;
+                    const int ty = t / g.tiles_x, tx = t - ty * g.tiles_x;
+                    const int col = 10 * tx - 1 + c, row = 10 * ty - py;
+                    const bool ok = L >= 1 && L <= 160 && (unsigned)col < (unsigned)a.Wout;
+                    eoff[2 * i + h] = row * a.Wout + col;
+                    erow[2 * i + h] = ok ? row : -(1 << 20);
+                }
+            }
+            typedef float floatx2 __attribute__((ext_vector_type(2)));
+            typedef unsigned uintx2 __attribute__((ext_vector_type(2)));
+#pragma unroll
+            for (int rc = 0; rc < 2; ++rc) {
+                const float bv = ebase[rc];
+                float y0[5][5], y1[5][5];
+#pragma unroll
+                for (int x = 0; x < 5; ++x) {
+                    float col[5];
+                    at6_5(zz[0][2 * rc][x], zz[1][2 * rc][x], zz[2][2 * rc][x], zz[3][2 * rc][x], zz[4][2 * rc][x], zz[5][2 * rc][x], col);
+#pragma unroll
+                    for (int dy = 0; dy < 5; ++dy) y0[dy][x] = col[dy] + bv;
+                    at6_5(zz[0][2 * rc + 1][x], zz[1][2 * rc + 1][x], zz[2][2 * rc + 1][x], zz[3][2 * rc + 1][x], zz[4][2 * rc + 1][x], zz[5][2 * rc + 1][x], col);
+#pragma unroll
+                    for (int dy = 0; dy < 5; ++dy) y1[dy][x] = col[dy] + bv;
+                }
+                const int chb = (int)(ch_off + (unsigned)(rc * HWo));
+#pragma unroll
+                for (int dy = 0; dy < 5; ++dy) {
+                    float* const wl = sb + 10 * j;
+                    wl[1] = y1[dy][0];
+#pragma unroll
+                    for (int x = 0; x < 4; ++x) *reinterpret_cast<floatx2*>(wl + 2 + 2 * x) = floatx2{y0[dy][x], y1[dy][x + 1]};
+                    wl[10] = y0[dy][4];
+                    float plo[6], phi[6];
+#pragma unroll
+                    for (int i = 0; i < 6; ++i) {
+                        const floatx2 pr = *reinterpret_cast<const floatx2*>(sb + 2 * (16 * i + j));
+                        plo[i] = pr.x, phi[i] = pr.y;
+                        asm volatile("" : "+v"(plo[i]), "+v"(phi[i]));
+                    }
+#pragma unroll
+                    for (int i = 0; i < 6; ++i) {
+                        const bool lo = (unsigned)(erow[2 * i] + 2 * dy) < (unsigned)a.Hout, hi = (unsigned)(erow[2 * i + 1] + 2 * dy) < (unsigned)a.Hout;
+                        const int olo = (chb + eoff[2 * i] + 2 * dy * a.Wout) * 4, ohi = (chb + eoff[2 * i + 1] + 2 * dy * a.Wout) * 4;
+                        if (lo && hi && ohi == olo + 4) {
+                            __builtin_amdgcn_raw_buffer_store_b64(uintx2{__builtin_bit_cast(unsigned, plo[i]), __builtin_bit_cast(unsigned, phi[i])}, rso, olo, 0, 0);
+                        } else {
+                            if (lo) __builtin_amdgcn_raw_buffer_store_b32(__builtin_bit_cast(unsigned, plo[i]), rso, olo, 0, 0);
+                            if (hi) __builtin_amdgcn_raw_buffer_store_b32(__builtin_bit_cast(unsigned, phi[i]), rso, ohi, 0, 0);
+                        }
+                    }
+                }
+                __builtin_amdgcn_sched_barrier(0);
+            }
+        }
+        __syncthreads();
+        if (tid < 32 && more) econst[(epar ^ 1) * 64 + tid] = pre_e;
+        epar ^= 1;
+    }
+    asm volatile("s_waitcnt vmcnt(0)" ::: "memory");
+}
+
+__global__ __launch_bounds__(NT) void conv_wino4u_kernel(const ConvArgs a, const Geo4u g, const float* const wimg) {
+    extern __shared__ __attribute__((aligned(16))) float smem[];
+    if (__builtin_amdgcn_readfirstlane(threadIdx.x >> 6) < 4) conv_wino4u_body<true>(a, g, wimg, smem);
+    else conv_wino4u_body<false>(a, g, wimg, smem);
+}
+
+__global__ void pack_wino4u_kernel(const float* __restrict__ w, float* __restrict__ out, int Cout, int Cin) {
+    const int ncobv = 2 * ((Cout + 31) / 32);
+    const long long n = 4ll * Cout * Cin;
+    for (long long i = blockIdx.x * (long long)blockDim.x + threadIdx.x; i < n; i += (long long)gridDim.x * blockDim.x) {
+        const int co = i % Cout;
+        const long long i1 = i / Cout;
+        const int ph = i1 & 3, ci = i1 >> 2;
+        const int py = ph >> 1, px = ph & 1;
+        float gk[3][3];
+        load_taps(w, Cin, co, ci, 0, gk);
+        float k2[2][3];
+#pragma unroll
+        for (int q = 0; q < 3; ++q) {
+            k2[0][q] = py ? gk[0][q] + gk[1][q] : gk[0][q];
+            k2[1][q] = py ? gk[2][q] : gk[1][q] + gk[2][q];
+        }
+        float t[6][2];
+#pragma unroll
+        for (int q = 0; q < 2; ++q) {
+            const float c0 = q == 0 ? (px ? k2[0][0] + k2[0][1] : k2[0][0]) : (px ? k2[0][2] : k2[0][1] + k2[0][2]);
+            const float c1 = q == 0 ? (px ? k2[1][0] + k2[1][1] : k2[1][0]) : (px ? k2[1][2] : k2[1][1] + k2[1][2]);
+            float o[6];
+            g6_2(c0, c1, o);
+#pragma unroll
+            for (int u = 0; u < 6; ++u) t[u][q] = o[u];
+        }
+        const int cc = ci >> 2, kk = ci & 3;
+        const int vcb = 2 * (co >> 5) + py, cb = (co & 31) >> 3, i16 = 2 * (co & 7) + px;
+        float* dst = out + ((long long)cc * ncobv + vcb) * U_FLOATS + cb * 256 + (kk * 16 + i16) * 4;
+#pragma unroll
+        for (int u = 0; u < 6; ++u) {
+            float o[6];
+            g6_2(t[u][0], t[u][1], o);
+#pragma unroll
+            for (int v = 0; v < 6; ++v) {
+                const int p = pos(u, v);
+                dst[(p >> 2) * 1024 + (p & 3)] = o[v];
+            }
+        }
+    }
+}
+
+}
+
+namespace idiff_detail {
+
+long long conv_wino4u_items(const ConvArgs& a, int ks, int mode, const float* wimg) {
+    if (ks != 3 || mode != IDIFF_CONV_UPSAMPLE2 || !wimg) return 0;
+    if (a.src1 || a.pro_a || a.res || a.vec || a.aux || a.stats) return 0;
+    if (a.Cout % 16 || a.Cin % 8 || a.Cin < 16) return 0;
+    if ((long long)a.Cin * a.Hin * a.Win * 4 >= (1ll << 31)) return 0;
+    if ((long long)a.Cout * a.Hout * a.Wout * 4 >= (1ll << 31)) return 0;
+    const int ncobv = 2 * ((a.Cout + 31) / 32);
+    if (144ll * a.Cin * ncobv * 64 + U_FLOATS * 4 >= (1ll << 31)) return 0;
+    if ((reinterpret_cast<uintptr_t>(wimg) & 15) != 0) return 0;
+    const int tiles_x = (a.Wout + 10) / 10, tiles_y = (a.Hout + 10) / 10;
+    const int maxq = (tiles_x + 30) / tiles_x < tiles_y - 1 ? (tiles_x + 30) / tiles_x : tiles_y - 1;
+    if (maxq > MAXQ) return 0;
+    return (long long)((tiles_x * tiles_y + NTILE - 1) / NTILE) * ncobv;
+}
+
+int launch_conv_wino4u(const ConvArgs& a, const float* wimg, hipStream_t st) {
+    const size_t lds = ((size_t)2 * R_FLOATS + 2 * V_FLOATS + 2 * U_FLOATS + 128 + NL * NT) * sizeof(float);
+    static idiff_dyn_lds_cache lds_cache;
+    if (const int rc = idiff_dyn_lds(lds_cache, conv_wino4u_kernel, lds, "conv2d(winograd4u)")) return rc;
+    int num_cu = 0;
+    if (!idiff_num_cu(&num_cu)) IDIFF_FAIL(IDIFF_E_HIP, "conv2d(winograd4u): cannot query the CU count");
+    Geo4u g;
+    g.ncobv = 2 * ((a.Cout + 31) / 32);
+    g.tiles_x = (a.Wout + 10) / 10;
+    g.tiles_y = (a.Hout + 10) / 10;
+    g.nruns = (g.tiles_x * g.tiles_y + NTILE - 1) / NTILE;
+    const long long total = (long long)a.B * g.nruns * g.ncobv;
+    if (total >= (1ll << 31)) IDIFF_FAIL(IDIFF_E_BADARG, "conv2d(winograd4u): grid too large");
+    g.total = (int)total;
+    const int grid = persistent_grid(g.total, num_cu);
+    hipLaunchKernelGGL(conv_wino4u_kernel, dim3(grid), dim3(NT), lds, st, a, g, wimg);
+    IDIFF_CHECK_LAUNCH("conv2d_fwd(winograd4u)");
+    return IDIFF_OK;
+}
+
+}
+
+extern "C" int idiff_pack_conv_weight_wino4u(const float* w, float* wwino4u, int Cout, int Cin, idiff_stream_t stream) {
+    IDIFF_CHECK_ARG(w && wwino4u && Cout > 0 && Cin > 0, "pack_conv_weight_wino4u: bad args");
+    IDIFF_CHECK_ARG(Cout % 16 == 0 && Cin % 8 == 0, "pack_conv_weight_wino4u: needs Cout %% 16 == 0 and Cin %% 8 == 0 (got %d, %d)", Cout, Cin);
+    if (Cout % 32) {
+        hipError_t e = hipMemsetAsync(wwino4u, 0, (size_t)144 * Cin * ((Cout + 31) / 32) * 32 * sizeof(float), (hipStream_t)stream);
+        if (e != hipSuccess) IDIFF_FAIL(IDIFF_E_HIP, "pack_conv_weight_wino4u: hipMemsetAsync: %s", hipGetErrorString(e));
+    }
+    const long long n = 4ll * Cout * Cin;
+    const int grid = (int)((n + 255) / 256 > 4096 ? 4096 : (n + 255) / 256);
+    hipLaunchKernelGGL(pack_wino4u_kernel, dim3(grid), dim3(256), 0, (hipStream_t)stream, w, wwino4u, Cout, Cin);
+    IDIFF_CHECK_LAUNCH("pack_conv_weight_wino4u");
+    return IDIFF_OK;
+}
diff --git a/instancediff_amd/csrc/wino_common.h b/instancediff_amd/csrc/wino_common.h
--- a/instancediff_amd/csrc/wino_common.h
+++ b/instancediff_amd/csrc/wino_common.h
@@ -72,6 +72,22 @@
     o[3] = (1.f / 24.f) * __builtin_fmaf(2.f, x1, t);
     o[4] = (1.f / 24.f) * __builtin_fmaf(-2.f, x1, t);
     o[5] = x2;
+}
+__device__ __forceinline__ void g6_2(float x0, float x1, float (&o)[6]) {
+    o[0] = 0.25f * x0;
+    o[1] = (-1.f / 6.f) * (x0 + x1);
+    o[2] = (-1.f / 6.f) * (x0 - x1);
+    o[3] = (1.f / 24.f) * __builtin_fmaf(2.f, x1, x0);
+    o[4] = (1.f / 24.f) * __builtin_fmaf(-2.f, x1, x0);
+    o[5] = x1;
+}
+__device__ __forceinline__ void at6_5(const float x0, const float x1, const float x2, const float x3, const float x4, const float x5, float (&o)[5]) {
+    const float s1 = x1 + x2, d1 = x1 - x2, s2 = x3 + x4, d2 = x3 - x4;
+    o[0] = (x0 + s1) + s2;
+    o[1] = __builtin_fmaf(2.f, d2, d1);
+    o[2] = __builtin_fmaf(4.f, s2, s1);
+    o[3] = __builtin_fmaf(8.f, d2, d1);
+    o[4] = __builtin_fmaf(16.f, s2, s1) + x5;
 }
 __device__ __forceinline__ void gt3(float m0, float m1, float m2, float m3, float m4, float m5, float (&o)[3]) {
     const float s12 = m1 + m2, d12 = m1 - m2, s34 = m3 + m4, d34 = m3 - m4;
diff --git a/instancediff_amd/models/modules/MSM_degEmb_Unet.py b/instancediff_amd/models/modules/MSM_degEmb_Unet.py
--- a/instancediff_amd/models/modules/MSM_degEmb_Unet.py
+++ b/instancediff_amd/models/modules/MSM_degEmb_Unet.py
@@ -56,6 +56,12 @@
     if ops.current_conv_operands() == "bf16" and tuple(conv.weight.shape[2:]) == (3, 3):
         return _PREP.get(("pk_bf16", conv), (conv.weight,), lambda: ops.pack_conv_weight(conv.weight.detach().contiguous(), bf16=True))
     return _PREP.get(("pk", conv), (conv.weight,), lambda: ops.pack_conv_weight(conv.weight.detach().contiguous()))
+
+
+def packed_subpixel(conv):
+    if ops.current_conv_operands() == "bf16":
+        return packed(conv)
+    return _PREP.get(("pk_subpixel", conv), (conv.weight,), lambda: ops.pack_conv_weight(conv.weight.detach().contiguous(), subpixel=True))
 
 
 def wT(lin):
@@ -520,7 +526,7 @@
         self.conv = nn.Conv2d(dim_in, dim_out, 3, padding=1)
 
     def run(self, x):
-        return ops.conv2d(x, packed(self.conv), self.conv.bias, 3, self.dim_out, mode=ops.CONV_UPSAMPLE2)
+        return ops.conv2d(x, packed_subpixel(self.conv), self.conv.bias, 3, self.dim_out, mode=ops.CONV_UPSAMPLE2)
 
 
 class SameConv(nn.Module):
diff --git a/instancediff_amd/ops.py b/instancediff_amd/ops.py
--- a/instancediff_amd/ops.py
+++ b/instancediff_amd/ops.py
@@ -64,6 +64,7 @@
 
 CONV_ALGO_DIRECT, CONV_ALGO_WINOGRAD, CONV_ALGO_STREAM1X1, CONV_ALGO_WINOGRAD4, CONV_ALGO_WINOGRAD4H, CONV_ALGO_X3 = 0, 1, 2, 3, 4, 5
 CONV_ALGO_BF16 = 6
+CONV_ALGO_WINOGRAD4U = 7
 _ALGO_REQUEST = threading.local()
 CONV_OPERANDS = ("f32", "bf16")
 _OPERANDS = threading.local()
@@ -132,9 +133,13 @@
         check(lib.idiff_pack_conv_weight_bf16(_p(w), out.bf16.data_ptr(), co, ci, tr, _stream()), "pack_conv_weight_bf16")
 
 
-def pack_conv_weight(w, transpose=False, bf16=False):
+def pack_conv_weight(w, transpose=False, bf16=False, subpixel=False):
     out = _alloc_conv_images(w, transpose, bf16)
     _fill_conv_images(out, w, transpose)
+    co, ci, k, _ = w.shape
+    if subpixel and not transpose and k == 3 and co % 16 == 0 and ci % 8 == 0 and ci >= 16:
+        out.wino4u = torch.empty((144 * ci * ((co + 31) // 32) * 32,), device=w.device, dtype=torch.float32)
+        check(_lib.load().idiff_pack_conv_weight_wino4u(_p(w), _p(out.wino4u), co, ci, _stream()), "pack_conv_weight_wino4u")
     return out
 
 
@@ -178,6 +183,9 @@
         wino4 = getattr(wpk, "wino4", None)
         if wino4 is not None:
             d.wwino4 = wino4.data_ptr()
+    wino4u = getattr(wpk, "wino4u", None)
+    if wino4u is not None and ks == 3 and mode == CONV_UPSAMPLE2:
+        d.wwino4u = wino4u.data_ptr()
     x3 = getattr(wpk, "x3", None)
     if x3 is not None and ks == 1 and mode in (CONV_NORMAL, CONV_UNSHUFFLE2):
         d.wx3 = x3.data_ptr()
```

After: 44.45 steps/s (median of 6 runs). No clear change (+0.7%).
